# congliuUvA/Clifford-Group-Equivariant-Simplicial-Message-Passing-Networks

Hardware: NVIDIA B200
Metric: simplices/sec fwd+bwd per CSMPN layer (higher is better)
Workload: dtype f32

## Files before the change

clifford-group-equivariant-simplicial-message-passing-networks_b200/csrc/tc_block.cuh:

```cuda
#pragma once
#include "tc_common.cuh"

namespace csmpn {
namespace tcb {
using namespace tc;

constexpr int kTile = 128;
constexpr int kThreads = 512;
constexpr float kInvSqrt2 = 0.70710678118654752440f;

constexpr uint32_t kKH = 2048;
constexpr uint32_t kPS = 2 * kKH + 16;

__host__ __device__ constexpr int round_up(int x, int m) { return (x + m - 1) / m * m; }
__host__ __device__ constexpr int64_t bpt_floats(int B, int64_t rows, int cp) {
  return ((rows + kTile - 1) / kTile) * (int64_t)B * cp * kTile;
}
__device__ __forceinline__ size_t bpt_off(int B, int cp, int64_t tile, int b, int c4, int r) {
  return ((((size_t)tile * B + b) * (cp >> 2) + c4) * kTile + r) * 4;
}

__device__ __forceinline__ float fast_rcp(float x) { float y; asm("rcp.approx.f32 %0, %1;" : "=f"(y) : "f"(x)); return y; }
__device__ __forceinline__ float fast_sqrt(float x) { float y; asm("sqrt.approx.f32 %0, %1;" : "=f"(y) : "f"(x)); return y; }
__device__ __forceinline__ float fast_ex2(float x) { float y; asm("ex2.approx.f32 %0, %1;" : "=f"(y) : "f"(x)); return y; }
__device__ __forceinline__ float fast_sigmoid(float v) { return fast_rcp(1.f + fast_ex2(-1.4426950408889634f * v)); }
__device__ __forceinline__ float fast_sas(float q) { return fast_sqrt(fast_sqrt(fmaf(q, q, kSmoothEps))); }

template <int DIM>
__device__ __forceinline__ void silu_gates(const float* y1, const float* a, const float* b, float* sg, float* inv) {
  using A = Alg<DIM>;
#pragma unroll
  for (int g = 0; g < A::G; ++g) inv[g] = 0.f;
#pragma unroll
  for (int i = 0; i < A::B; ++i) inv[A::grade_of(i)] = fmaf(y1[i], y1[i], inv[A::grade_of(i)]);
  inv[0] = y1[0];
#pragma unroll
  for (int g = 0; g < A::G; ++g) sg[g] = fast_sigmoid(fmaf(a[g], inv[g], b[g]));
}

template <int DIM>
__device__ __forceinline__ void norm_factors(const float* xr, const float* s, float* q, float* nrm, float* rinv) {
  using A = Alg<DIM>;
#pragma unroll
  for (int g = 0; g < A::G; ++g) q[g] = 0.f;
#pragma unroll
  for (int i = 0; i < A::B; ++i) q[A::grade_of(i)] = fmaf(xr[i], xr[i], q[A::grade_of(i)]);
#pragma unroll
  for (int g = 0; g < A::G; ++g) {
    nrm[g] = fast_sas(q[g]);
    rinv[g] = fast_rcp(fmaf(s[g], nrm[g] - 1.f, 1.f) + kEps);
  }
}

template <int DIM>
__device__ __forceinline__ float mv_sumsq(const float* x) {
  float Q = 0.f;
#pragma unroll
  for (int i = 0; i < Alg<DIM>::B; ++i) Q = fmaf(x[i], x[i], Q);
  return Q;
}

struct WJob {
  uint8_t* img0;
  const float* w;
  int c_out, c_in, row0;
};
template <int DIM, bool TRANS, int NJ>
__device__ __forceinline__ void stage_weight_jobs(const WJob (&j)[NJ], int njobs, uint32_t img_bytes, int rows_p, int cols_p,
                                                  uint8_t* zero_base, uint32_t zero_bytes) {
  static_assert(NJ == 1 || NJ == 2, "one or two weights per call");
  constexpr int G = Alg<DIM>::G, U = 4;
  const int lane = threadIdx.x & 31, warp = threadIdx.x >> 5, nwarps = blockDim.x >> 5;
  const int rl = lane >> 2, cl = lane & 3;
  const WJob& j0 = j[0];
  const WJob& j1 = j[NJ - 1];
  const bool two = NJ == 2 && njobs > 1;
  const int R0 = TRANS ? j0.c_in : j0.c_out, C0 = TRANS ? j0.c_out : j0.c_in;
  const int R1 = TRANS ? j1.c_in : j1.c_out, C1 = TRANS ? j1.c_out : j1.c_in;
  const int ncb0 = (C0 + 3) >> 2, ncb1 = (C1 + 3) >> 2;
  const int nb0 = ((R0 + 7) >> 3) * ncb0, nb1 = two ? ((R1 + 7) >> 3) * ncb1 : 0;
  const int total = nb0 + nb1;
  auto decode = [&](int wb, bool& sj, int& row, int& col) -> bool {
    if (wb >= total) return false;
    sj = wb >= nb0;
    if (sj) wb -= nb0;
    const int ncb = sj ? ncb1 : ncb0;
    const int rb = wb / ncb, cb = wb - rb * ncb;
    row = rb * 8 + rl;
    col = cb * 4 + cl;
    return row < (sj ? R1 : R0) && col < (sj ? C1 : C0);
  };
  auto fetch = [&](int wb, float* v) {
#pragma unroll
    for (int g = 0; g < G; ++g) v[g] = 0.f;
    bool sj;
    int row, col;
    if (!decode(wb, sj, row, col)) return;
    const int o = TRANS ? col : row, i = TRANS ? row : col;
    const float* src = (sj ? j1.w : j0.w) + ((size_t)o * (sj ? j1.c_in : j0.c_in) + i) * G;
    if (G == 4 && (reinterpret_cast<uintptr_t>(src) & 15) == 0) {
      const float4 x = __ldg(reinterpret_cast<const float4*>(src));
      v[0] = x.x; v[1] = x.y; v[2] = x.z; v[G - 1] = x.w;
    } else {
#pragma unroll
      for (int g = 0; g < G; ++g) v[g] = __ldg(src + g);
    }
  };
  auto put = [&](int wb, const float* v) {
    bool sj;
    int row, col;
    if (!decode(wb, sj, row, col)) return;
    const int r = (sj ? j1.row0 : j0.row0) + row;
    if (r >= rows_p || col >= cols_p) return;
    uint8_t* dst = (sj ? j1.img0 : j0.img0) + plane_off(rows_p, r, col);
#pragma unroll
    for (int g = 0; g < G; ++g) {
      const float hi = tf32_hi(v[g]);
      *reinterpret_cast<float*>(dst + (size_t)(g * 2 + 0) * img_bytes) = hi;
      *reinterpret_cast<float*>(dst + (size_t)(g * 2 + 1) * img_bytes) = v[g] - hi;
    }
  };
  float x[U][G];
#pragma unroll
  for (int u = 0; u < U; ++u) fetch(warp + u * nwarps, x[u]);
  for (uint32_t i = threadIdx.x; i < (zero_bytes >> 4); i += blockDim.x)
    reinterpret_cast<float4*>(zero_base)[i] = make_float4(0.f, 0.f, 0.f, 0.f);
  __syncthreads();
  for (int base = 0; base < total; base += U * nwarps) {
    float nx[U][G];
    const int nbase = base + U * nwarps;
    if (nbase < total) {
#pragma unroll
      for (int u = 0; u < U; ++u) fetch(nbase + warp + u * nwarps, nx[u]);
    }
#pragma unroll
    for (int u = 0; u < U; ++u) put(base + warp + u * nwarps, x[u]);
    if (nbase < total) {
#pragma unroll
      for (int u = 0; u < U; ++u) {
#pragma unroll
        for (int g = 0; g < G; ++g) x[u][g] = nx[u][g];
      }
    }
  }
}
template <int DIM, bool TRANS>
__device__ __forceinline__ void stage_weight_images(uint8_t* img0, uint32_t img_bytes, const float* __restrict__ w, int c_out,
                                                    int c_in, int rows_p, int cols_p) {
  const WJob j[1] = {{img0, w, c_out, c_in, 0}};
  stage_weight_jobs<DIM, TRANS, 1>(j, 1, img_bytes, rows_p, cols_p, img0, (uint32_t)Alg<DIM>::G * 2u * img_bytes);
}

__device__ __forceinline__ uint64_t chunk_desc(uint32_t half_saddr, int b) {
  return smem_desc(half_saddr + (uint32_t)b * kPS, kKH, 128u);
}

constexpr bool kTf32Truncates = true;
constexpr int kRing = 3;
constexpr int kPipeBars = 3 * kRing + 1;
constexpr int kConvWarps = kThreads / 32 - 1;
constexpr int kConv = kConvWarps * 32;
struct Pipe {
  uint8_t* raw;
  uint8_t* lo;
  uint64_t* load_bar;
  uint64_t* slot_bar;
  uint64_t* full_bar;
  uint64_t* lo_bar;
  uint32_t half;
  __device__ __forceinline__ uint8_t* slot(int q) const { return raw + (size_t)(q % kRing) * half; }
  __device__ __forceinline__ void init(uint8_t* base, uint64_t* bars, uint32_t half_bytes) {
    raw = base; lo = base + (size_t)kRing * half_bytes; half = half_bytes;
    load_bar = bars; slot_bar = bars + kRing; full_bar = bars + 2 * kRing; lo_bar = bars + 3 * kRing;
    if (threadIdx.x == 0) {
      for (int i = 0; i < kPipeBars; ++i) mbar_init(&bars[i], (i >= 2 * kRing && i < 3 * kRing) ? kConvWarps : 1);
      mbar_fence_init();
    }
  }
  __device__ __forceinline__ void conv_done(int q) const {
    fence_async_smem();
    fence_before_sync();
    __syncwarp();
    if ((threadIdx.x & 31) == 0) mbar_arrive(&full_bar[q % kRing]);
  }
  __device__ __forceinline__ void wait_full(int q) const {
    mbar_wait(&full_bar[q % kRing], (q / kRing) & 1);
    fence_after_sync();
  }
};

template <int DIM>
__host__ __device__ constexpr uint32_t wunit_bytes(int rows) { return (uint32_t)Alg<DIM>::G * 2u * (uint32_t)rows * 32u; }

template <int B>
__device__ __forceinline__ void issue_chunk_load_w(const Pipe& p, int q, const float* bpt, int cp, int64_t tile, int kc,
                                                   const uint8_t* wsrc, uint32_t wbytes) {
  const int lane = threadIdx.x & 31;
  uint64_t* bar = &p.load_bar[q % kRing];
  if (lane == 0) mbar_arrive_expect_tx(bar, (bpt ? B * 4096u : 0u) + wbytes);
  __syncwarp();
  if (bpt && lane < B) bulk_g2s(p.slot(q) + lane * kPS, bpt + bpt_off(B, cp, tile, lane, 2 * kc, 0), 4096u, bar);
  if (lane == B) bulk_g2s(p.slot(q) + B * kPS, wsrc, wbytes, bar);
}

struct WPrepArgs {
  const float *w0, *w1;
  int stack, trans, n_real, k_real0, k_real1, np, npass, nk0, nk1;
  float* out;
};
template <int DIM>
__global__ void tc_weight_images_kernel(WPrepArgs a) {
  constexpr int G = Alg<DIM>::G;
  const int R = a.stack ? 2 * a.np : a.np;
  const int nk = a.nk0 + (a.stack ? 0 : a.nk1);
  const int64_t total = (int64_t)a.npass * nk * G * 2 * R * 8;
  for (int64_t e = blockIdx.x * (int64_t)blockDim.x + threadIdx.x; e < total; e += (int64_t)gridDim.x * blockDim.x) {
    const int c = (int)(e & 3), r = (int)((e >> 2) % R), cu = (int)((e / (4 * R)) & 1), hl = (int)((e / (8 * R)) & 1);
    const int g = (int)((e / (16 * R)) % G);
    const int u = (int)(e / ((int64_t)16 * R * G)), ps = u / nk, kc = u % nk;
    const int second_k = (!a.stack && kc >= a.nk0) ? 1 : 0;
    const int k = (second_k ? kc - a.nk0 : kc) * 8 + cu * 4 + c;
    const int k_real = second_k ? a.k_real1 : a.k_real0;
    const float* w = a.stack ? (r < a.np ? a.w0 : a.w1) : (second_k ? a.w1 : a.w0);
    const int n = ps * a.np + (a.stack ? r % a.np : r);
    float x = 0.f;
    if (w && n < a.n_real && k < k_real) x = a.trans ? w[((size_t)k * a.n_real + n) * G + g] : w[((size_t)n * k_real + k) * G + g];
    const float hi = tf32_hi(x);
    a.out[e] = hl ? x - hi : hi;
  }
}
template <int DIM>
__host__ inline int64_t weight_image_floats(int stack, int np, int npass, int nk_total) {
  return (int64_t)npass * nk_total * Alg<DIM>::G * 2 * (stack ? 2 * np : np) * 8;
}

template <int B>
__device__ __forceinline__ void issue_chunk_load(const Pipe& p, int q, const float* bpt, int cp, int64_t tile, int kc) {
  const int lane = threadIdx.x & 31;
  uint64_t* bar = &p.load_bar[q % kRing];
  if (lane == 0) mbar_arrive_expect_tx(bar, B * 4096u);
  __syncwarp();
  if (lane < B) bulk_g2s(p.slot(q) + lane * kPS, bpt + bpt_off(B, cp, tile, lane, 2 * kc, 0), 4096u, bar);
}
template <int B>
__device__ __forceinline__ void split_chunk(const Pipe& p, int q) {
  uint8_t* hi = p.slot(q);
  constexpr int TOT = B * 2 * kTile;
  constexpr int N = (TOT + kConv - 1) / kConv;
  const int ct = (int)threadIdx.x - 32;
  float4 l[N];
#pragma unroll
  for (int i = 0; i < N; ++i) {
    const int it = ct + i * kConv;
    if (it < TOT) {
      const int r = it & (kTile - 1), kh = (it >> 7) & 1, b = it >> 8;
      const uint32_t off = b * kPS + kh * kKH + r * 16;
      const float4 x = *reinterpret_cast<const float4*>(hi + off);
      float4 h;
      split4(x, h, l[i]);
      if (!kTf32Truncates) *reinterpret_cast<float4*>(hi + off) = h;
    }
  }
  if (q >= 1) mbar_wait(p.lo_bar, (q - 1) & 1);
#pragma unroll
  for (int i = 0; i < N; ++i) {
    const int it = ct + i * kConv;
    if (it < TOT) {
      const int r = it & (kTile - 1), kh = (it >> 7) & 1, b = it >> 8;
      *reinterpret_cast<float4*>(p.lo + b * kPS + kh * kKH + r * 16) = l[i];
    }
  }
  p.conv_done(q);
}
template <int DIM>
__device__ __forceinline__ void issue_chunk_mma(const Pipe& p, int q, uint32_t tbase, uint32_t ncols, bool accumulate,
                                                const uint8_t* wimg0, uint32_t img_bytes, int s0, int nsets, uint32_t set_bytes,
                                                uint32_t w_rows, int ks, int n0, uint32_t idesc) {
  using A = Alg<DIM>;
  constexpr int B = A::B;
  const uint64_t a_hi = chunk_desc(smem_addr(p.slot(q)), 0), a_lo = chunk_desc(smem_addr(p.lo), 0);
  const uint64_t w0 = smem_desc(smem_addr(wimg0) + (uint32_t)s0 * set_bytes + 2u * ks * w_rows * 16u + (uint32_t)n0 * 16u,
                                w_rows * 16u, 128u);
  const uint64_t img16 = img_bytes >> 4, set16 = set_bytes >> 4;
  constexpr uint64_t ps16 = kPS >> 4;
#pragma unroll
  for (int s = 0; s < 2; ++s) {
    if (s < nsets) {
#pragma unroll
      for (int b = 0; b < B; ++b)
        mma_tf32_w(tbase + (uint32_t)(s * B + b) * ncols, a_lo + b * ps16, w0 + s * set16 + (2 * A::grade_of(b)) * img16, idesc,
                 accumulate);
    }
  }
  mma_commit_w(p.lo_bar);
#pragma unroll
  for (int s = 0; s < 2; ++s) {
    if (s < nsets) {
#pragma unroll
      for (int b = 0; b < B; ++b) {
        const uint64_t wd = w0 + s * set16 + (2 * A::grade_of(b)) * img16;
        const uint32_t d = tbase + (uint32_t)(s * B + b) * ncols;
        mma_tf32_w(d, a_hi + b * ps16, wd, idesc, 1);
        mma_tf32_w(d, a_hi + b * ps16, wd + img16, idesc, 1);
      }
    }
  }
  mma_commit_w(&p.slot_bar[q % kRing]);
}

}
}
```

clifford-group-equivariant-simplicial-message-passing-networks_b200/csrc/tc_block_bwd.cu:

```cuda
#include <utility>
#include <vector>

#include "tc_block.cuh"

namespace csmpn {
namespace tcb {

struct EwArgs {
  int64_t rows;
  int tiles, C, Cp;
  const float* gy;
  int gy_bpt;
  const int32_t* gy_rows;
  int64_t gy_stride;
  const float *o, *xr, *y2, *y1, *dy2;
  const float *la, *wp, *na, *sa, *sb;
  float *d, *dxr, *dy2p, *dy1;
  float* partial;
};

template <int DIM>
__device__ __forceinline__ void load_mv_bpt(float* v, const float* t, int Cp, int64_t tile, int c4, int r, int j) {
  constexpr int B = Alg<DIM>::B;
#pragma unroll
  for (int b = 0; b < B; ++b) v[b] = t[bpt_off(B, Cp, tile, b, c4, r) + j];
}
template <int DIM>
__device__ __forceinline__ void store_mv_bpt(float* t, const float* v, int Cp, int64_t tile, int c4, int r, int j) {
  constexpr int B = Alg<DIM>::B;
#pragma unroll
  for (int b = 0; b < B; ++b) t[bpt_off(B, Cp, tile, b, c4, r) + j] = v[b];
}

__device__ __forceinline__ void cp_async4(float* dst_smem, const float* src) {
  asm volatile("cp.async.ca.shared.global [%0], [%1], 4;" ::"r"(smem_addr(dst_smem)), "l"(src) : "memory");
}
__device__ __forceinline__ void cp_async_commit() { asm volatile("cp.async.commit_group;" ::: "memory"); }
template <int N>
__device__ __forceinline__ void cp_async_wait() { asm volatile("cp.async.wait_group %0;" ::"n"(N) : "memory"); }

__device__ __forceinline__ void cp_async16(float* dst_smem, const float* src) {
  asm volatile("cp.async.cg.shared.global [%0], [%1], 16;" ::"r"(smem_addr(dst_smem)), "l"(src) : "memory");
}
template <int DIM>
__device__ __forceinline__ void prefetch_mv_bpt(float* st, const float* t, int Cp, int64_t tile, int c4, int r0, int lane) {
  constexpr int B = Alg<DIM>::B;
#pragma unroll
  for (int k = lane; k < B * 8; k += 32) {
    const int b = k >> 3, row = k & 7;
    cp_async16(st + (b * 8 + row) * 4, t + bpt_off(B, Cp, tile, b, c4, r0 + row));
  }
}
template <int DIM>
__device__ __forceinline__ void read_stage(float* v, const float* st, int lane) {
#pragma unroll
  for (int b = 0; b < Alg<DIM>::B; ++b) v[b] = st[b * 32 + lane];
}

template <int DIM, int CP, int CPT>
__global__ void __launch_bounds__(CP * 8, CP <= 32 ? 2 : 1) tc_b1_kernel(EwArgs a) {
  using A = Alg<DIM>;
  constexpr int B = A::B, G = A::G, P = A::P, NP = P + G + 2;
  constexpr int NSLAB = CPT / CP;
  static_assert(CPT % CP == 0, "wide blocks are whole slabs");
  extern __shared__ float sm[];
  constexpr int nw = CP >> 2, nt = CP * 8;
  float* part1 = sm;
  float* part2 = part1 + nw * kTile;
  float* inv_mu_s = part2 + nw * kTile;
  float* dmu_s = inv_mu_s + kTile;
  float* stage = dmu_s + kTile;
  const int tid = threadIdx.x, c4l = tid >> 5, lane = tid & 31, j = lane & 3, rr = lane >> 2;
  const int c4 = (NSLAB > 1 ? (int)blockIdx.y * nw : 0) + c4l;
  const int ch = c4 * 4 + j, C = a.C;
  constexpr int Cp = CPT;
  const bool ch_ok = ch < C;
  float la = ch_ok ? a.la[ch] : 0.f, wv[P], sn[G];
#pragma unroll
  for (int q = 0; q < P; ++q) wv[q] = ch_ok ? a.wp[ch * P + q] : 0.f;
#pragma unroll
  for (int g = 0; g < G; ++g) sn[g] = ch_ok ? sigmoidf_(a.na[ch * G + g]) : 0.f;
  float g_w[P], g_na[G], g_la = 0.f, g_bl = 0.f;
#pragma unroll
  for (int q = 0; q < P; ++q) g_w[q] = 0.f;
#pragma unroll
  for (int g = 0; g < G; ++g) g_na[g] = 0.f;

  constexpr int kIt = kTile / 16;
  constexpr int kIt1 = NSLAB * kIt;
  float* stage_w = stage + (size_t)c4l * (2 * 4 * B * 32);
  auto stage_of = [&](int s, int tensor) { return stage_w + (size_t)(s * 4 + tensor) * B * 32; };
  auto prefetch = [&](int64_t unit, int it, int s) {
    const int64_t tile = unit >> 1;
    const int r0 = (int)(unit & 1) * (kTile / 2) + (it & (kIt - 1)) * 8, r = r0 + rr;
    const int c4x = it < kIt1 ? (it / kIt) * nw + c4l : c4;
    const int chx = c4x * 4 + j;
    __syncwarp();
    prefetch_mv_bpt<DIM>(stage_of(s, 0), a.o, Cp, tile, c4x, r0, lane);
    if (a.gy_bpt) {
      prefetch_mv_bpt<DIM>(stage_of(s, 1), a.gy, Cp, tile, c4x, r0, lane);
    } else {
      float* dst = stage_of(s, 1) + lane;
      if (chx < C && tile * kTile + r < a.rows) {
        const int64_t grow = a.gy_rows ? (int64_t)__ldg(a.gy_rows + tile * kTile + r) : tile * kTile + r;
        const float* src = a.gy + (size_t)grow * a.gy_stride + (size_t)chx * B;
#pragma unroll
        for (int b = 0; b < B; ++b) cp_async4(dst + b * 32, src + b);
      } else {
#pragma unroll
        for (int b = 0; b < B; ++b) dst[b * 32] = 0.f;
      }
    }
    if (it >= kIt1) {
      prefetch_mv_bpt<DIM>(stage_of(s, 2), a.y2, Cp, tile, c4, r0, lane);
      prefetch_mv_bpt<DIM>(stage_of(s, 3), a.xr, Cp, tile, c4, r0, lane);
    }
    cp_async_commit();
  };

  const int64_t n_units = 2 * (int64_t)a.tiles;
  int seq = 0;
  if ((int64_t)blockIdx.x < n_units) prefetch(blockIdx.x, 0, 0);
  for (int64_t unit = blockIdx.x; unit < n_units; unit += gridDim.x) {
    const int64_t tile = unit >> 1;
    const int rbase = (int)(unit & 1) * (kTile / 2);
    const int64_t row0 = tile * kTile;
#pragma unroll 1
    for (int it = 0; it < kIt1 + kIt; ++it, ++seq) {
      if (it + 1 < kIt1 + kIt) prefetch(unit, it + 1, (seq + 1) & 1);
      else if (unit + gridDim.x < n_units) prefetch(unit + gridDim.x, 0, (seq + 1) & 1);
      else cp_async_commit();
      cp_async_wait<1>();
      __syncwarp();
      const int s = seq & 1;
      const int r = rbase + (it & (kIt - 1)) * 8 + rr;
      const bool ok = ch_ok && row0 + r < a.rows;
      if (it < kIt1) {
        const int chx = ((it / kIt) * nw + c4l) * 4 + j;
        const bool okx = chx < C && row0 + r < a.rows;
        const float lax = NSLAB > 1 ? (chx < C ? a.la[chx] : 0.f) : la;
        float o[B], dy[B];
        read_stage<DIM>(o, stage_of(s, 0), lane);
        read_stage<DIM>(dy, stage_of(s, 1), lane);
        float dot = 0.f;
#pragma unroll
        for (int b = 0; b < B; ++b) dot = fmaf(dy[b], o[b], dot);
        float nu = okx ? fast_sas(mv_sumsq<DIM>(o)) : 0.f;
        float dt = okx ? lax * dot : 0.f;
        nu += __shfl_xor_sync(0xffffffffu, nu, 1); dt += __shfl_xor_sync(0xffffffffu, dt, 1);
        nu += __shfl_xor_sync(0xffffffffu, nu, 2); dt += __shfl_xor_sync(0xffffffffu, dt, 2);
        if (j == 0) {
          if (NSLAB > 1 && it >= kIt) { part1[c4l * kTile + r] += nu; part2[c4l * kTile + r] += dt; }
          else { part1[c4l * kTile + r] = nu; part2[c4l * kTile + r] = dt; }
        }
        if (it == kIt1 - 1) {
          __syncthreads();
          if (tid < kTile / 2) {
            const int r2 = rbase + tid;
            float s1 = 0.f, s2 = 0.f;
            for (int w = 0; w < nw; ++w) { s1 += part1[w * kTile + r2]; s2 += part2[w * kTile + r2]; }
            const float inv_mu = 1.f / (s1 / (float)C + kEps);
            inv_mu_s[r2] = inv_mu;
            dmu_s[r2] = -s2 * inv_mu * inv_mu / (float)C;
          }
          __syncthreads();
        }
        continue;
      }
      float dd[B];
      {
        float o[B];
        read_stage<DIM>(o, stage_of(s, 0), lane);
        read_stage<DIM>(dd, stage_of(s, 1), lane);
        const float inv_mu = inv_mu_s[r];
        float dot = 0.f;
#pragma unroll
        for (int b = 0; b < B; ++b) dot = fmaf(dd[b], o[b], dot);
        if (ok) g_la = fmaf(dot, inv_mu, g_la);
        const float Q = mv_sumsq<DIM>(o);
        const float nu = fast_sas(Q);
        const float k1 = la * inv_mu * kInvSqrt2;
        const float k2 = dmu_s[r] * Q * fast_rcp(nu * nu * nu) * kInvSqrt2;
#pragma unroll
        for (int b = 0; b < B; ++b) dd[b] = ok ? fmaf(k1, dd[b], k2 * o[b]) : 0.f;
      }
      store_mv_bpt<DIM>(a.d, dd, Cp, tile, c4, r, j);
      g_bl += dd[0];
      float y2[B], xr[B];
      read_stage<DIM>(y2, stage_of(s, 2), lane);
      read_stage<DIM>(xr, stage_of(s, 3), lane);
      float q[G], nrm[G], rinv[G], xn[B], dxn[B], dy2[B];
      norm_factors<DIM>(xr, sn, q, nrm, rinv);
#pragma unroll
      for (int b = 0; b < B; ++b) { xn[b] = xr[b] * rinv[A::grade_of(b)]; dy2[b] = 0.f; dxn[b] = 0.f; }
      A::template wgp_bwd<false>(y2, xn, wv, dd, nullptr, dy2, dxn, g_w);
      store_mv_bpt<DIM>(a.dy2p, dy2, Cp, tile, c4, r, j);
      float t[G], coef[G];
#pragma unroll
      for (int g = 0; g < G; ++g) t[g] = 0.f;
#pragma unroll
      for (int b = 0; b < B; ++b) t[A::grade_of(b)] = fmaf(dxn[b], xr[b], t[A::grade_of(b)]);
#pragma unroll
      for (int g = 0; g < G; ++g) {
        const float ddn = -t[g] * rinv[g] * rinv[g];
        g_na[g] = fmaf(ddn * (nrm[g] - 1.f), sn[g] * (1.f - sn[g]), g_na[g]);
        coef[g] = ddn * sn[g] * q[g] * fast_rcp(nrm[g] * nrm[g] * nrm[g]);
      }
#pragma unroll
      for (int b = 0; b < B; ++b) dxn[b] = fmaf(dxn[b], rinv[A::grade_of(b)], coef[A::grade_of(b)] * xr[b]);
      store_mv_bpt<DIM>(a.dxr, dxn, Cp, tile, c4, r, j);
    }
  }
  cp_async_wait<0>();
  auto red = [&](float v) {
    v += __shfl_xor_sync(0xffffffffu, v, 4);
    v += __shfl_xor_sync(0xffffffffu, v, 8);
    v += __shfl_xor_sync(0xffffffffu, v, 16);
    return v;
  };
  float* out = a.partial + ((size_t)blockIdx.x * C + (ch_ok ? ch : 0)) * NP;
#pragma unroll
  for (int q = 0; q < P; ++q) { const float v = red(g_w[q]); if (rr == 0 && ch_ok) out[q] = v; }
#pragma unroll
  for (int g = 0; g < G; ++g) { const float v = red(g_na[g]); if (rr == 0 && ch_ok) out[P + g] = v; }
  { const float v = red(g_la); if (rr == 0 && ch_ok) out[P + G] = v; }
  { const float v = red(g_bl); if (rr == 0 && ch_ok) out[P + G + 1] = v; }
}

template <int DIM, int CP, int CPT>
__global__ void __launch_bounds__(CP * 8, CP <= 32 ? 2 : 1) tc_b3_kernel(EwArgs a) {
  using A = Alg<DIM>;
  constexpr int B = A::B, G = A::G, NP = 2 * G + 1;
  extern __shared__ float sm[];
  constexpr int nt = CP * 8;
  float* stage = sm;
  const int tid = threadIdx.x, c4l = tid >> 5, lane = tid & 31, j = lane & 3, rr = lane >> 2;
  const int c4 = (CPT > CP ? (int)blockIdx.y * (CP >> 2) : 0) + c4l;
  const int ch = c4 * 4 + j, C = a.C;
  constexpr int Cp = CPT;
  const bool ch_ok = ch < C;
  float sa[G], sb[G], g_sa[G], g_sb[G], g_b1 = 0.f;
#pragma unroll
  for (int g = 0; g < G; ++g) {
    sa[g] = ch_ok ? a.sa[ch * G + g] : 0.f;
    sb[g] = ch_ok ? a.sb[ch * G + g] : 0.f;
    g_sa[g] = 0.f; g_sb[g] = 0.f;
  }
  constexpr int kIt = kTile / 16;
  float* stage_w = stage + (size_t)c4l * (2 * 2 * B * 32);
  auto stage_of = [&](int s, int tensor) { return stage_w + (size_t)(s * 2 + tensor) * B * 32; };
  auto prefetch = [&](int64_t unit, int it, int s) {
    const int64_t tile = unit >> 1;
    const int r0 = (int)(unit & 1) * (kTile / 2) + it * 8;
    __syncwarp();
    prefetch_mv_bpt<DIM>(stage_of(s, 0), a.y1, Cp, tile, c4, r0, lane);
    prefetch_mv_bpt<DIM>(stage_of(s, 1), a.dy2, Cp, tile, c4, r0, lane);
    cp_async_commit();
  };
  const int64_t n_units = 2 * (int64_t)a.tiles;
  int seq = 0;
  if ((int64_t)blockIdx.x < n_units) prefetch(blockIdx.x, 0, 0);
  for (int64_t unit = blockIdx.x; unit < n_units; unit += gridDim.x) {
    const int64_t tile = unit >> 1;
    const int rbase = (int)(unit & 1) * (kTile / 2);
    const int64_t row0 = tile * kTile;
#pragma unroll 1
    for (int it = 0; it < kIt; ++it, ++seq) {
      if (it + 1 < kIt) prefetch(unit, it + 1, (seq + 1) & 1);
      else if (unit + gridDim.x < n_units) prefetch(unit + gridDim.x, 0, (seq + 1) & 1);
      else cp_async_commit();
      cp_async_wait<1>();
      __syncwarp();
      const int s = seq & 1;
      const int r = rbase + it * 8 + rr;
      const bool ok = ch_ok && row0 + r < a.rows;
      float y1[B], dy[B], sg[G], inv[G], t[G], ds[G];
      read_stage<DIM>(y1, stage_of(s, 0), lane);
      read_stage<DIM>(dy, stage_of(s, 1), lane);
      silu_gates<DIM>(y1, sa, sb, sg, inv);
#pragma unroll
      for (int g = 0; g < G; ++g) t[g] = 0.f;
#pragma unroll
      for (int b = 0; b < B; ++b) t[A::grade_of(b)] = fmaf(dy[b], y1[b], t[A::grade_of(b)]);
#pragma unroll
      for (int g = 0; g < G; ++g) {
        ds[g] = ok ? t[g] * sg[g] * (1.f - sg[g]) : 0.f;
        g_sa[g] = fmaf(ds[g], inv[g], g_sa[g]);
        g_sb[g] += ds[g];
      }
#pragma unroll
      for (int b = 0; b < B; ++b) {
        const int g = A::grade_of(b);
        const float dinv = (g == 0) ? 1.f : 2.f * y1[b];
        dy[b] = ok ? fmaf(sg[g], dy[b], ds[g] * sa[g] * dinv) : 0.f;
      }
      g_b1 += dy[0];
      store_mv_bpt<DIM>(a.dy1, dy, Cp, tile, c4, r, j);
    }
  }
  cp_async_wait<0>();
  auto red = [&](float v) {
    v += __shfl_xor_sync(0xffffffffu, v, 4);
    v += __shfl_xor_sync(0xffffffffu, v, 8);
    v += __shfl_xor_sync(0xffffffffu, v, 16);
    return v;
  };
  float* out = a.partial + ((size_t)blockIdx.x * C + (ch_ok ? ch : 0)) * NP;
#pragma unroll
  for (int g = 0; g < G; ++g) { const float v = red(g_sa[g]); if (rr == 0 && ch_ok) out[g] = v; }
#pragma unroll
  for (int g = 0; g < G; ++g) { const float v = red(g_sb[g]); if (rr == 0 && ch_ok) out[G + g] = v; }
  { const float v = red(g_b1); if (rr == 0 && ch_ok) out[2 * G] = v; }
}

struct GemmArgs {
  int64_t rows;
  int tiles;
  const float* src[2];
  int cp[2], nk[2];
  const float* w[2];
  int wk[2], wn;
  int n16;
  int kmax;
  const float* addend;
  float* out;
  int out_bpt;
  const float *y1, *sa, *sb;
  float* partial;
  int C;
  const float* wimg;
  int np;
};

__device__ __forceinline__ float warp_transpose_reduce16(float (&v)[16], int lane) {
#pragma unroll
  for (int step = 8; step >= 1; step >>= 1) {
    const bool up = (lane & step) != 0;
#pragma unroll
    for (int i = 0; i < step; ++i) {
      const float send = up ? v[i] : v[i + step];
      const float keep = up ? v[i + step] : v[i];
      v[i] = keep + __shfl_xor_sync(0xffffffffu, send, step);
    }
  }
  return v[0] + __shfl_xor_sync(0xffffffffu, v[0], 16);
}
__device__ __forceinline__ float warp_sum(float v) {
#pragma unroll
  for (int o = 16; o >= 1; o >>= 1) v += __shfl_xor_sync(0xffffffffu, v, o);
  return v;
}

template <int DIM, bool SILU, bool ST>
__global__ void __launch_bounds__(kThreads, 1) tc_bgemm_kernel(GemmArgs a) {
  using A = Alg<DIM>;
  constexpr int B = A::B, G = A::G, NPS = 2 * G + 1;
  static_assert(2 * NPS <= 18, "two channels' SiLU gradients are reduced as 16 + 2 values");
  extern __shared__ __align__(1024) uint8_t smem[];
  const int tid = threadIdx.x, warp = uniform_warp_idx(), lane = tid & 31;
  const int nmax = ST ? a.np : (512 / B) / 16 * 16;
  const uint32_t wunit = ST ? wunit_bytes<DIM>(nmax) : 0u;
  const uint32_t half = B * kPS + wunit;
  const uint32_t img = ST ? (uint32_t)nmax * 32u : (uint32_t)a.n16 * a.kmax * 4;
  const uint32_t set_bytes = ST ? 0u : G * 2 * img;
  uint8_t* wimg = smem + (size_t)kRing * half + B * kPS;
  const int nsets = a.src[1] ? 2 : 1;
  uint64_t* bars = reinterpret_cast<uint64_t*>(wimg + (size_t)nsets * set_bytes);
  uint32_t* tmem_slot = reinterpret_cast<uint32_t*>(bars + kPipeBars);
  float* sa_s = reinterpret_cast<float*>(tmem_slot + 4);
  float* sb_s = sa_s + a.n16 * G;
  Pipe p;
  p.init(smem, bars, half);
  if (SILU) {
    for (int i = tid; i < a.n16 * G; i += kThreads) {
      sa_s[i] = (i < a.C * G) ? a.sa[i] : 0.f;
      sb_s[i] = (i < a.C * G) ? a.sb[i] : 0.f;
    }
  }
  float acc[4][2];
#pragma unroll
  for (int it = 0; it < 4; ++it) {
#pragma unroll
    for (int pr = 0; pr < 2; ++pr) acc[it][pr] = 0.f;
  }
  const int npass = (a.n16 + nmax - 1) / nmax;
  const int nk = a.nk[0] + a.nk[1];
  const int per_tile = npass * nk;
  const int my_tiles = (a.tiles - (int)blockIdx.x + (int)gridDim.x - 1) / (int)gridDim.x;
  const int total_chunks = my_tiles * per_tile;
  auto issue = [&](int qq) {
    const int64_t tile = (int64_t)blockIdx.x + (int64_t)(qq / per_tile) * gridDim.x;
    const int kc = (qq % per_tile) % nk;
    const int s = kc < a.nk[0] ? 0 : 1;
    if constexpr (ST) {
      const uint8_t* wsrc = reinterpret_cast<const uint8_t*>(a.wimg) + (size_t)(qq % per_tile) * wunit;
      issue_chunk_load_w<B>(p, qq, a.src[s], a.cp[s], tile, s ? kc - a.nk[0] : kc, wsrc, wunit);
    } else {
      issue_chunk_load<B>(p, qq, a.src[s], a.cp[s], tile, s ? kc - a.nk[0] : kc);
    }
  };
  int q = 0, loaded = 0;
  if (warp == 0) for (; loaded < kRing - 1 && loaded < total_chunks; ++loaded) issue(loaded);
  const uint32_t need = (uint32_t)B * (a.n16 < nmax ? a.n16 : nmax);
  const uint32_t tcols = need <= 32 ? 32 : need <= 64 ? 64 : need <= 128 ? 128 : need <= 256 ? 256 : 512;
  if (warp == 0) tmem_alloc(tmem_slot, tcols);
  if (!ST) {
    {
    const WJob wj[2] = {{wimg, a.w[0], a.wk[0], a.wn, 0}, {wimg + set_bytes, a.w[nsets - 1], a.wk[nsets - 1], a.wn, 0}};
    stage_weight_jobs<DIM, true, 2>(wj, nsets, img, a.n16, a.kmax, wimg, (uint32_t)nsets * set_bytes);
  }
  }
  fence_async_smem();
  fence_before_sync();
  __syncthreads();
  fence_after_sync();
  const uint32_t tbase = *tmem_slot;
  const uint32_t lane_base = (warp & 3) * 32;
  const bool wide_ok = aligned32(a.out);
  for (int t = 0; t < my_tiles; ++t) {
    const int64_t tile = (int64_t)blockIdx.x + (int64_t)t * gridDim.x;
    const int64_t row0 = tile * kTile;
    for (int ps = 0; ps < npass; ++ps) {
      const int n0 = ps * nmax;
      const int Np = (a.n16 - n0) < nmax ? (a.n16 - n0) : nmax;
      const uint32_t idesc = idesc_tf32(kTile, Np, false, false);
      for (int kc = 0; kc < nk; ++kc, ++q) {
        if (warp == 0) {
          p.wait_full(q);
          if (loaded == q + kRing - 1 && loaded < total_chunks) {
            if (q >= 1) mbar_wait(&p.slot_bar[(q - 1) % kRing], ((q - 1) / kRing) & 1);
            issue(loaded);
            ++loaded;
          }
          if constexpr (ST) {
            mbar_wait(&p.load_bar[q % kRing], (q / kRing) & 1);
            issue_chunk_mma<DIM>(p, q, tbase, Np, kc > 0, p.slot(q) + B * kPS, img, 0, 1, 0, nmax, 0, 0, idesc);
          } else {
            const int s = kc < a.nk[0] ? 0 : 1;
            issue_chunk_mma<DIM>(p, q, tbase, Np, kc > 0, wimg, img, s, 1, set_bytes, a.n16, s ? kc - a.nk[0] : kc, n0, idesc);
          }
        } else {
          mbar_wait(&p.load_bar[q % kRing], (q / kRing) & 1);
          split_chunk<B>(p, q);
        }
      }
      const int r = lane_base + lane;
      const bool row_ok = row0 + r < a.rows;
      float4 ad[B];
      if (a.addend && (warp >> 2) < (Np >> 2)) {
#pragma unroll
        for (int b = 0; b < B; ++b) ad[b] = *reinterpret_cast<const float4*>(a.addend + bpt_off(B, a.n16, tile, b, (n0 >> 2) + (warp >> 2), r));
      }
      mbar_wait(&p.slot_bar[(q - 1) % kRing], ((q - 1) / kRing) & 1);
      fence_after_sync();
      if (warp == 0) for (; loaded < q + kRing && loaded < total_chunks; ++loaded) issue(loaded);
      for (int c4 = warp >> 2; c4 < (Np >> 2); c4 += 4) {
        float v[B][4];
#pragma unroll
        for (int b = 0; b < B; ++b) tmem_ld4(tmem_at(tbase, lane_base, b * Np + c4 * 4), v[b]);
        tmem_wait_ld();
        const int gc4 = (n0 >> 2) + c4;
        if (a.addend) {
#pragma unroll
          for (int b = 0; b < B; ++b) {
            v[b][0] += ad[b].x; v[b][1] += ad[b].y; v[b][2] += ad[b].z; v[b][3] += ad[b].w;
          }
          if (c4 + 4 < (Np >> 2)) {
#pragma unroll
            for (int b = 0; b < B; ++b) ad[b] = *reinterpret_cast<const float4*>(a.addend + bpt_off(B, a.n16, tile, b, gc4 + 4, r));
          }
        }
        if constexpr (SILU) {
          const int it = c4 >> 2;
#pragma unroll
          for (int pr = 0; pr < 2; ++pr) {
            float2 y1v[B];
#pragma unroll
            for (int b = 0; b < B; ++b)
              y1v[b] = *reinterpret_cast<const float2*>(a.y1 + bpt_off(B, a.n16, tile, b, gc4, r) + 2 * pr);
            float vals[16], t0 = 0.f, t1 = 0.f;
#pragma unroll
            for (int i = 0; i < 16; ++i) vals[i] = 0.f;
#pragma unroll
            for (int jj = 0; jj < 2; ++jj) {
              const int j = 2 * pr + jj, ch = gc4 * 4 + j;
              float y1[B], dy[B], sg[G], inv[G], tg[G], ds[G];
#pragma unroll
              for (int b = 0; b < B; ++b) {
                y1[b] = jj == 0 ? y1v[b].x : y1v[b].y;
                dy[b] = v[b][j];
              }
              const float* sa = sa_s + ch * G;
              silu_gates<DIM>(y1, sa, sb_s + ch * G, sg, inv);
#pragma unroll
              for (int g = 0; g < G; ++g) tg[g] = 0.f;
#pragma unroll
              for (int b = 0; b < B; ++b) tg[A::grade_of(b)] = fmaf(dy[b], y1[b], tg[A::grade_of(b)]);
              const bool ok = row_ok && ch < a.C;
              float gv[NPS];
#pragma unroll
              for (int g = 0; g < G; ++g) {
                ds[g] = ok ? tg[g] * sg[g] * (1.f - sg[g]) : 0.f;
                gv[g] = ds[g] * inv[g];
                gv[G + g] = ds[g];
              }
#pragma unroll
              for (int b = 0; b < B; ++b) {
                const int g = A::grade_of(b);
                const float dinv = (g == 0) ? 1.f : 2.f * y1[b];
                v[b][j] = ok ? fmaf(sg[g], dy[b], ds[g] * sa[g] * dinv) : 0.f;
              }
              gv[2 * G] = v[0][j];
#pragma unroll
              for (int k = 0; k < NPS; ++k) {
                const int idx = jj * NPS + k;
                if (idx < 16) vals[idx] = gv[k];
                else if (idx == 16) t0 = gv[k];
                else t1 = gv[k];
              }
            }
            const float s16 = warp_transpose_reduce16(vals, lane);
            t0 = warp_sum(t0);
            t1 = warp_sum(t1);
            const float mine = lane < 16 ? s16 : lane == 16 ? t0 : lane == 17 ? t1 : 0.f;
#pragma unroll
            for (int q4 = 0; q4 < 4; ++q4) {
              if (q4 == it) acc[q4][pr] += mine;
            }
          }
        }
        if (a.out_bpt) {
#pragma unroll
          for (int b = 0; b < B; ++b) {
            float4 x = make_float4(v[b][0], v[b][1], v[b][2], v[b][3]);
            if (!row_ok) x = make_float4(0.f, 0.f, 0.f, 0.f);
            *reinterpret_cast<float4*>(a.out + bpt_off(B, a.n16, tile, b, gc4, r)) = x;
          }
        } else if (row_ok) {
#pragma unroll
          for (int jj = 0; jj < 4; ++jj) {
            const int n = gc4 * 4 + jj;
            if (n >= a.wn) continue;
            float* dst = a.out + ((size_t)(row0 + r) * a.wn + n) * B;
            if constexpr (B == 8) {
              if (wide_ok) {
                float w8[8];
#pragma unroll
                for (int b = 0; b < 8; ++b) w8[b] = v[b][jj];
                st_global_v8(dst, w8);
                continue;
              }
            }
#pragma unroll
            for (int h = 0; h < B / 4; ++h)
              *reinterpret_cast<float4*>(dst + 4 * h) = make_float4(v[4 * h][jj], v[4 * h + 1][jj], v[4 * h + 2][jj], v[4 * h + 3][jj]);
          }
        }
      }
      fence_before_sync();
    }
  }
  fence_before_sync();
  __syncthreads();
  if (warp == 0) tmem_dealloc(tbase, tcols);
  if constexpr (SILU) {
    float* red = reinterpret_cast<float*>(p.lo);
#pragma unroll
    for (int it = 0; it < 4; ++it) {
#pragma unroll
      for (int pr = 0; pr < 2; ++pr) {
        float* dst = red + ((warp * 4 + it) * 2 + pr) * 18;
        if (lane < 18) dst[lane] = acc[it][pr];
      }
    }
    __syncthreads();
    for (int e = tid; e < a.C * NPS; e += kThreads) {
      const int ch = e / NPS, k = e - ch * NPS;
      const int c4 = ch >> 2, j = ch & 3, cg = c4 & 3, it = c4 >> 2, pr = j >> 1, idx = (j & 1) * NPS + k;
      float sum = 0.f;
#pragma unroll
      for (int q4 = 0; q4 < 4; ++q4) sum += red[(((cg * 4 + q4) * 4 + it) * 2 + pr) * 18 + idx];
      a.partial[((size_t)blockIdx.x * a.C + ch) * NPS + k] = sum;
    }
  }
}

template <int DIM, bool SILU>
__global__ void __launch_bounds__(kThreads, 1) tc_bgemmdb_kernel(GemmArgs a) {
  using A = Alg<DIM>;
  constexpr int B = A::B, G = A::G, NPS = 2 * G + 1;
  constexpr int kUnits = 6;
  extern __shared__ __align__(1024) uint8_t smem[];
  const int tid = threadIdx.x, warp = uniform_warp_idx(), lane = tid & 31;
  const uint32_t img = (uint32_t)a.n16 * a.kmax * 4;
  const uint32_t set_bytes = G * 2 * img;
  uint8_t* wimg = smem + (kRing + 1) * B * kPS;
  const int nsets = a.src[1] ? 2 : 1;
  uint64_t* bars = reinterpret_cast<uint64_t*>(wimg + (size_t)nsets * set_bytes);
  uint32_t* tmem_slot = reinterpret_cast<uint32_t*>(bars + kPipeBars);
  float* sa_s = reinterpret_cast<float*>(tmem_slot + 4);
  float* sb_s = sa_s + a.n16 * G;
  Pipe p;
  p.init(smem, bars, B * kPS);
  if (SILU) {
    for (int i = tid; i < a.n16 * G; i += kThreads) {
      sa_s[i] = (i < a.C * G) ? a.sa[i] : 0.f;
      sb_s[i] = (i < a.C * G) ? a.sb[i] : 0.f;
    }
  }
  float acc[kUnits][2];
#pragma unroll
  for (int u = 0; u < kUnits; ++u) { acc[u][0] = 0.f; acc[u][1] = 0.f; }
  const int nk = a.nk[0] + a.nk[1];
  const int my_tiles = (a.tiles - (int)blockIdx.x + (int)gridDim.x - 1) / (int)gridDim.x;
  const int total_chunks = my_tiles * nk;
  auto issue = [&](int qq) {
    const int64_t tile = (int64_t)blockIdx.x + (int64_t)(qq / nk) * gridDim.x;
    const int kc = qq % nk;
    const int s = kc < a.nk[0] ? 0 : 1;
    issue_chunk_load<B>(p, qq, a.src[s], a.cp[s], tile, s ? kc - a.nk[0] : kc);
  };
  int q = 0, loaded = 0;
  if (warp == 0) for (; loaded < kRing - 1 && loaded < total_chunks; ++loaded) issue(loaded);
  const int Np = a.n16;
  const uint32_t bufcols = (uint32_t)B * Np;
  const uint32_t need = 2 * bufcols;
  const uint32_t tcols = need <= 32 ? 32 : need <= 64 ? 64 : need <= 128 ? 128 : need <= 256 ? 256 : 512;
  if (warp == 0) tmem_alloc(tmem_slot, tcols);
  {
    const WJob wj[2] = {{wimg, a.w[0], a.wk[0], a.wn, 0}, {wimg + set_bytes, a.w[nsets - 1], a.wk[nsets - 1], a.wn, 0}};
    stage_weight_jobs<DIM, true, 2>(wj, nsets, img, a.n16, a.kmax, wimg, (uint32_t)nsets * set_bytes);
  }
  fence_async_smem();
  fence_before_sync();
  __syncthreads();
  fence_after_sync();
  const uint32_t tbase = *tmem_slot;
  const uint32_t idesc = idesc_tf32(kTile, Np, false, false);
  const uint32_t lane_base = (warp & 3) * 32;
  const int r = lane_base + lane;
  const bool wide_ok = aligned32(a.out);
  const int n_c4 = Np >> 2;

  auto epilogue_unit = [&](int64_t tile, int c4, uint32_t tb) {
    const int64_t row0 = tile * kTile;
    const bool row_ok = row0 + r < a.rows;
    float v[B][4];
#pragma unroll
    for (int b = 0; b < B; ++b) tmem_ld4(tmem_at(tb, lane_base, b * Np + c4 * 4), v[b]);
    if (a.addend) {
      float4 ad[B];
#pragma unroll
      for (int b = 0; b < B; ++b) ad[b] = *reinterpret_cast<const float4*>(a.addend + bpt_off(B, a.n16, tile, b, c4, r));
      tmem_wait_ld();
#pragma unroll
      for (int b = 0; b < B; ++b) {
        v[b][0] += ad[b].x; v[b][1] += ad[b].y; v[b][2] += ad[b].z; v[b][3] += ad[b].w;
      }
    } else {
      tmem_wait_ld();
    }
    if constexpr (SILU) {
      const int u = c4 / 3;
#pragma unroll
      for (int pr = 0; pr < 2; ++pr) {
        float2 y1v[B];
#pragma unroll
        for (int b = 0; b < B; ++b)
          y1v[b] = *reinterpret_cast<const float2*>(a.y1 + bpt_off(B, a.n16, tile, b, c4, r) + 2 * pr);
        float vals[16], t0 = 0.f, t1 = 0.f;
#pragma unroll
        for (int i = 0; i < 16; ++i) vals[i] = 0.f;
#pragma unroll
        for (int jj = 0; jj < 2; ++jj) {
          const int j = 2 * pr + jj, ch = c4 * 4 + j;
          float y1[B], dy[B], sg[G], inv[G], tg[G], ds[G];
#pragma unroll
          for (int b = 0; b < B; ++b) {
            y1[b] = jj == 0 ? y1v[b].x : y1v[b].y;
            dy[b] = v[b][j];
          }
          const float* sa = sa_s + ch * G;
          silu_gates<DIM>(y1, sa, sb_s + ch * G, sg, inv);
#pragma unroll
          for (int g = 0; g < G; ++g) tg[g] = 0.f;
#pragma unroll
          for (int b = 0; b < B; ++b) tg[A::grade_of(b)] = fmaf(dy[b], y1[b], tg[A::grade_of(b)]);
          const bool ok = row_ok && ch < a.C;
          float gv[NPS];
#pragma unroll
          for (int g = 0; g < G; ++g) {
            ds[g] = ok ? tg[g] * sg[g] * (1.f - sg[g]) : 0.f;
            gv[g] = ds[g] * inv[g];
            gv[G + g] = ds[g];
          }
#pragma unroll
          for (int b = 0; b < B; ++b) {
            const int g = A::grade_of(b);
            const float dinv = (g == 0) ? 1.f : 2.f * y1[b];
            v[b][j] = ok ? fmaf(sg[g], dy[b], ds[g] * sa[g] * dinv) : 0.f;
          }
          gv[2 * G] = v[0][j];
#pragma unroll
          for (int k = 0; k < NPS; ++k) {
            const int idx = jj * NPS + k;
            if (idx < 16) vals[idx] = gv[k];
            else if (idx == 16) t0 = gv[k];
            else t1 = gv[k];
          }
        }
        const float s16 = warp_transpose_reduce16(vals, lane);
        t0 = warp_sum(t0);
        t1 = warp_sum(t1);
        const float mine = lane < 16 ? s16 : lane == 16 ? t0 : lane == 17 ? t1 : 0.f;
#pragma unroll
        for (int k = 0; k < kUnits; ++k) {
          if (k == u) acc[k][pr] += mine;
        }
      }
    }
    if (a.out_bpt) {
#pragma unroll
      for (int b = 0; b < B; ++b) {
        float4 x = make_float4(v[b][0], v[b][1], v[b][2], v[b][3]);
        if (!row_ok) x = make_float4(0.f, 0.f, 0.f, 0.f);
        *reinterpret_cast<float4*>(a.out + bpt_off(B, a.n16, tile, b, c4, r)) = x;
      }
    } else if (row_ok) {
#pragma unroll
      for (int jj = 0; jj < 4; ++jj) {
        const int n = c4 * 4 + jj;
        if (n >= a.wn) continue;
        float* dst = a.out + ((size_t)(row0 + r) * a.wn + n) * B;
        if constexpr (B == 8) {
          if (wide_ok) {
            float w8[8];
#pragma unroll
            for (int b = 0; b < 8; ++b) w8[b] = v[b][jj];
            st_global_v8(dst, w8);
            continue;
          }
        }
#pragma unroll
        for (int h = 0; h < B / 4; ++h)
          *reinterpret_cast<float4*>(dst + 4 * h) = make_float4(v[4 * h][jj], v[4 * h + 1][jj], v[4 * h + 2][jj], v[4 * h + 3][jj]);
      }
    }
  };
  int64_t pend_tile = -1;
  int pend_c4 = 0, pend_q = 0;
  uint32_t pend_tb = 0;
  bool pend_ready = false;
  auto epilogue_step = [&]() {
    if (warp < 4 || pend_tile < 0) return;
    if (!pend_ready) {
      mbar_wait(&p.slot_bar[pend_q % kRing], (pend_q / kRing) & 1);
      fence_after_sync();
      pend_ready = true;
    }
    if (pend_c4 < n_c4) {
      epilogue_unit(pend_tile, pend_c4, pend_tb);
      pend_c4 += 3;
    }
    if (pend_c4 >= n_c4) { pend_tile = -1; fence_before_sync(); }
  };

  for (int t = 0; t < my_tiles; ++t) {
    const int64_t tile = (int64_t)blockIdx.x + (int64_t)t * gridDim.x;
    const uint32_t tb = tbase + (uint32_t)(t & 1) * bufcols;
    for (int kc = 0; kc < nk; ++kc, ++q) {
      if (warp == 0) {
        p.wait_full(q);
        if (loaded == q + kRing - 1 && loaded < total_chunks) {
          if (q >= 1) mbar_wait(&p.slot_bar[(q - 1) % kRing], ((q - 1) / kRing) & 1);
          issue(loaded);
          ++loaded;
        }
        const int s = kc < a.nk[0] ? 0 : 1;
        issue_chunk_mma<DIM>(p, q, tb, Np, kc > 0, wimg, img, s, 1, set_bytes, a.n16, s ? kc - a.nk[0] : kc, 0, idesc);
      } else {
        mbar_wait(&p.load_bar[q % kRing], (q / kRing) & 1);
        split_chunk<B>(p, q);
        epilogue_step();
      }
    }
    while (warp >= 4 && pend_tile >= 0) epilogue_step();
    pend_tile = tile; pend_c4 = (warp >> 2) - 1; pend_q = q - 1; pend_tb = tb; pend_ready = false;
  }
  while (warp >= 4 && pend_tile >= 0) epilogue_step();
  fence_before_sync();
  __syncthreads();
  if (warp == 0) tmem_dealloc(tbase, tcols);
  if constexpr (SILU) {
    float* red = reinterpret_cast<float*>(p.lo);
#pragma unroll
    for (int u = 0; u < kUnits; ++u) {
#pragma unroll
      for (int pr = 0; pr < 2; ++pr) {
        float* dst = red + ((warp * kUnits + u) * 2 + pr) * 18;
        if (lane < 18) dst[lane] = acc[u][pr];
      }
    }
    __syncthreads();
    for (int e = tid; e < a.C * NPS; e += kThreads) {
      const int ch = e / NPS, k = e - ch * NPS;
      const int c4 = ch >> 2, j = ch & 3, g3 = c4 % 3, u = c4 / 3, pr = j >> 1, idx = (j & 1) * NPS + k;
      float sum = 0.f;
#pragma unroll
      for (int q4 = 0; q4 < 4; ++q4) sum += red[((((g3 + 1) * 4 + q4) * kUnits + u) * 2 + pr) * 18 + idx];
      a.partial[((size_t)blockIdx.x * a.C + ch) * NPS + k] = sum;
    }
  }
}

struct DwArgs {
  int64_t rows;
  int tiles;
  const float *a0, *a1, *bsrc;
  int cpa, cpb;
  int cpa_total;
  int a_c4;
  int cpb_total;
  int b_c4;
  int M;
  float* partial;
  long long* dbg;
};
long long*& debug_buffer();
#ifdef CSMPN_DEBUG_TOOLS
#define DW_STAMP(code)                                                                       \
  do {                                                                                       \
    if (TL && a.dbg && blockIdx.x == 0 && (tid == 0 || tid == 32) && dbg_n < 250) {          \
      a.dbg[(tid ? 512 : 0) + 2 * dbg_n] = (code);                                           \
      a.dbg[(tid ? 512 : 0) + 2 * dbg_n + 1] = clock64();                                    \
      ++dbg_n;                                                                               \
    }                                                                                        \
  } while (0)
#else
#define DW_STAMP(code) do { } while (0)
#endif

constexpr int kDwRows = 64;
constexpr int kDwLand = 2;
constexpr uint32_t kLand = kTile * 16;

template <int DIM, bool TL>
__global__ void __launch_bounds__(256, 1) tc_dw_kernel(DwArgs a) {
  using A = Alg<DIM>;
  constexpr int B = A::B, G = A::G;
  extern __shared__ __align__(1024) uint8_t smem[];
  const int tid = threadIdx.x, warp = uniform_warp_idx(), lane = tid & 31;
  [[maybe_unused]] int dbg_n = 0;
  const int ca4 = a.cpa >> 2;
  const int na4 = (a.a1 ? 2 : 1) * ca4;
  const int nb4 = a.cpb >> 2;
  const int n4 = na4 + nb4;
  const int ga = a.M / 32, gb = (a.cpb + 31) / 32;
  const uint32_t grp = kDwRows * 128;
  const uint32_t op_bytes = 2u * (ga + gb) * grp;
  uint8_t* ops = smem;
  uint8_t* land = ops + 2 * (size_t)op_bytes;
  const uint32_t land_bytes = (uint32_t)n4 * kLand;
  uint64_t* bars = reinterpret_cast<uint64_t*>(land + (size_t)kDwLand * land_bytes);
  uint64_t* load_bar = bars;
  uint64_t* op_bar = bars + kDwLand;
  uint64_t* full_bar = bars + kDwLand + 2;
  uint32_t* tmem_slot = reinterpret_cast<uint32_t*>(bars + kDwLand + 4);
  constexpr int kConvWarps = 7;
  for (uint32_t i = tid; i < (2 * op_bytes) >> 4; i += 256) reinterpret_cast<float4*>(smem)[i] = make_float4(0.f, 0.f, 0.f, 0.f);
  if (tid == 0) {
    for (int i = 0; i < kDwLand + 2; ++i) mbar_init(&bars[i], 1);
    mbar_init(&full_bar[0], kConvWarps);
    mbar_init(&full_bar[1], kConvWarps);
    mbar_fence_init();
  }
  const bool merged = a.M == 64;
  const uint32_t ncol = merged ? 2u * gb * 32u : (uint32_t)a.cpb;
  const uint32_t need = (uint32_t)G * ncol;
  const uint32_t tcols = need <= 32 ? 32 : need <= 64 ? 64 : need <= 128 ? 128 : need <= 256 ? 256 : 512;
  if (warp == 0) tmem_alloc(tmem_slot, tcols);
  fence_async_smem();
  fence_before_sync();
  __syncthreads();
  fence_after_sync();
  const uint32_t tbase = *tmem_slot;
  const uint32_t idesc = merged ? idesc_tf32(128, (int)ncol, true, true) : idesc_tf32(a.M, a.cpb, true, true);
  const int my_tiles = (a.tiles - (int)blockIdx.x + (int)gridDim.x - 1) / (int)gridDim.x;
  const int steps = my_tiles * B * 2;
  if (warp == 0) {
    const int units = steps >> 1;
    auto issue = [&](int lu) {
      const int64_t tile = (int64_t)blockIdx.x + (int64_t)(lu / B) * gridDim.x;
      const int b = lu % B;
      uint8_t* dst = land + (size_t)(lu % kDwLand) * land_bytes;
      uint64_t* bar = &load_bar[lu % kDwLand];
      if (lane == 0) {
        mbar_arrive_expect_tx(bar, (uint32_t)n4 * kLand);
        bulk_g2s(dst, a.a0 + bpt_off(B, a.cpa_total, tile, b, a.a_c4, 0), (uint32_t)ca4 * kLand, bar);
        if (a.a1) bulk_g2s(dst + (size_t)ca4 * kLand, a.a1 + bpt_off(B, a.cpa_total, tile, b, a.a_c4, 0), (uint32_t)ca4 * kLand, bar);
        bulk_g2s(dst + (size_t)na4 * kLand, a.bsrc + bpt_off(B, a.cpb_total, tile, b, a.b_c4, 0), (uint32_t)nb4 * kLand, bar);
      }
      __syncwarp();
    };
    int loaded = 0;
    for (; loaded < kDwLand && loaded < units; ++loaded) issue(loaded);
    uint32_t grade_used = 0;
    for (int st = 0; st < steps; ++st) {
      const int b = (st >> 1) % B, g = A::grade_of(b);
      DW_STAMP(30);
      mbar_wait(&full_bar[st & 1], (st >> 1) & 1);
      fence_after_sync();
      DW_STAMP(31);
      const uint8_t* op_a = ops + (size_t)(st & 1) * op_bytes;
      const uint8_t* op_b = op_a + 2 * (size_t)ga * grp;
      const uint64_t a_hi = desc_mn32b(smem_addr(op_a), grp, 0), a_lo = a_hi + ((uint64_t)ga * grp >> 4);
      const uint64_t b_hi = desc_mn32b(smem_addr(op_b), grp, 0), b_lo = b_hi + ((uint64_t)gb * grp >> 4);
      const uint32_t dcol = tbase + (uint32_t)g * ncol;
      const uint32_t acc = (grade_used >> g) & 1;
      if (merged) {
#pragma unroll
        for (int ks = 0; ks < kDwRows / 8; ++ks) mma_tf32_w(dcol, a_hi + ks * 64, b_hi + ks * 64, idesc, ks == 0 ? acc : 1u);
      } else {
#pragma unroll
        for (int ks = 0; ks < kDwRows / 8; ++ks) {
          mma_tf32_w(dcol, a_hi + ks * 64, b_hi + ks * 64, idesc, ks == 0 ? acc : 1u);
          mma_tf32_w(dcol, a_hi + ks * 64, b_lo + ks * 64, idesc, 1);
          mma_tf32_w(dcol, a_lo + ks * 64, b_hi + ks * 64, idesc, 1);
        }
      }
      mma_commit_w(&op_bar[st & 1]);
      __syncwarp();
      DW_STAMP(32);
      if ((st & 1) && loaded < units) { issue(loaded); ++loaded; }
      DW_STAMP(33);
      grade_used |= 1u << g;
    }
  } else {
    const int ct = tid - 32, nconv = kConvWarps * 32;
    for (int st = 0; st < steps; ++st) {
      const int lu = st >> 1, rh = st & 1;
      DW_STAMP(40);
      mbar_wait(&load_bar[lu % kDwLand], (lu / kDwLand) & 1);
      DW_STAMP(41);
      if (st >= 2) mbar_wait(&op_bar[st & 1], ((st - 2) >> 1) & 1);
      DW_STAMP(42);
      const uint8_t* src = land + (size_t)(lu % kDwLand) * land_bytes + (uint32_t)rh * (kDwRows * 16);
      uint8_t* op_a = ops + (size_t)(st & 1) * op_bytes;
      uint8_t* op_b = op_a + 2 * (size_t)ga * grp;
      for (int it = ct; it < kDwRows * n4; it += nconv) {
        const int pr = it >> 7, w = it & 127, q = w & 7, g8 = w >> 3;
        const int swap = g8 >> 3, r = ((g8 & 7) << 3) + q;
        const int u = 2 * pr + ((q >> 2) ^ swap);
        const float4 x = *reinterpret_cast<const float4*>(src + (uint32_t)u * kLand + r * 16);
        float4 h, l;
        split4(x, h, l);
        const bool isb = u >= na4;
        const int cc = (isb ? u - na4 : u) * 4;
        uint8_t* base = isb ? op_b : op_a;
        const int ng = isb ? gb : ga;
        const uint32_t off = (uint32_t)(cc >> 5) * grp + mn32b_off(r, cc & 31);
        *reinterpret_cast<float4*>(base + off) = h;
        *reinterpret_cast<float4*>(base + (size_t)ng * grp + off) = l;
      }
      fence_async_smem();
      __syncwarp();
      if (lane == 0) mbar_arrive(&full_bar[st & 1]);
      DW_STAMP(43);
    }
  }
  uint32_t grade_used = 0;
  for (int st = 0; st < steps; ++st) grade_used |= 1u << A::grade_of((st >> 1) % B);
  if (steps > 0) mbar_wait(&op_bar[(steps - 1) & 1], ((steps - 1) >> 1) & 1);
  fence_after_sync();
  if (warp < 4 && merged) {
    const int R = warp * 32 + lane, m = R & 63;
    float* out = a.partial + ((size_t)blockIdx.x * 2 + (R >> 6)) * G * 64 * a.cpb;
    for (int g = 0; g < G; ++g) {
      const bool used = steps > 0 && ((grade_used >> g) & 1);
      for (int n = 0; n < a.cpb; n += 4) {
        float v[4] = {0.f, 0.f, 0.f, 0.f}, w[4] = {0.f, 0.f, 0.f, 0.f};
        if (used) {
          tmem_ld4(tmem_at(tbase, warp * 32, g * ncol + n), v);
          tmem_ld4(tmem_at(tbase, warp * 32, g * ncol + gb * 32 + n), w);
          tmem_wait_ld();
        }
        *reinterpret_cast<float4*>(out + ((size_t)g * 64 + m) * a.cpb + n) = make_float4(v[0] + w[0], v[1] + w[1], v[2] + w[2], v[3] + w[3]);
      }
    }
  } else if (warp < 4) {
    float* out = a.partial + (size_t)blockIdx.x * G * a.M * a.cpb;
    const int m = warp * 32 + lane;
    for (int g = 0; g < G; ++g) {
      const bool used = steps > 0 && ((grade_used >> g) & 1);
      for (int n = 0; n < a.cpb; n += 4) {
        float v[4] = {0.f, 0.f, 0.f, 0.f};
        if (used) {
          tmem_ld4(tmem_at(tbase, warp * 32, g * a.cpb + n), v);
          tmem_wait_ld();
        }
        *reinterpret_cast<float4*>(out + ((size_t)g * a.M + m) * a.cpb + n) = make_float4(v[0], v[1], v[2], v[3]);
      }
    }
  }
  fence_before_sync();
  __syncthreads();
  if (warp == 0) tmem_dealloc(tbase, tcols);
}

struct FinalJob {
  const float* in;
  float* out;
  int parts;
  int64_t stride;
  int kind;
  int n;
  int G, M, N, m0, co, ci;
  int ci_tot, i0, o0;
};
constexpr int kFinalJobs = 14;
struct FinalJobs { FinalJob j[kFinalJobs]; int count; };

__global__ void __launch_bounds__(256) tc_final_kernel(FinalJobs jobs) {
  __shared__ float red[16][17];
  const int e = threadIdx.x & 15, pg = threadIdx.x >> 4;
  int64_t idx = (int64_t)blockIdx.x * 16 + e;
  float s = 0.f;
  float* outp = nullptr;
  for (int k = 0; k < jobs.count; ++k) {
    const FinalJob& jb = jobs.j[k];
    if (idx < jb.n) {
      if (jb.out) {
        size_t src, dst;
        if (jb.kind == 0) {
          src = dst = (size_t)idx;
        } else {
          const int i = (int)(idx % jb.ci), o = (int)((idx / jb.ci) % jb.co), g = (int)(idx / ((int64_t)jb.ci * jb.co));
          src = ((size_t)g * jb.M + jb.m0 + o) * jb.N + i;
          dst = ((size_t)(jb.o0 + o) * jb.ci_tot + jb.i0 + i) * jb.G + g;
        }
        const float* in = jb.in + src;
#pragma unroll 4
        for (int p = pg; p < jb.parts; p += 16) s += in[(size_t)p * jb.stride];
        outp = jb.out + dst;
      }
      break;
    }
    idx -= jb.n;
  }
  red[pg][e] = s;
  __syncthreads();
  if (pg == 0 && outp) {
    float t = 0.f;
#pragma unroll
    for (int i = 0; i < 16; ++i) t += red[i][e];
    *outp = t;
  }
}

template <int DIM>
size_t gemm_smem(int nsets, int n16, int kmax, bool silu = false) {
  constexpr int B = Alg<DIM>::B, G = Alg<DIM>::G;
  return (size_t)(kRing + 1) * B * kPS + (size_t)nsets * G * 2 * n16 * kmax * 4 + 128 + (silu ? (size_t)2 * n16 * G * 4 : 0);
}
inline bool fuse_silu_adjoint() {
  const char* e = getenv("CSMPN_TC_FUSE_SILU");
  return e && e[0] == '1';
}
template <int DIM>
size_t dw_smem(int M, int na4, int cpb) {
  const int ga = M / 32, gb = (cpb + 31) / 32;
  return (size_t)2 * 2 * (ga + gb) * kDwRows * 128 + (size_t)kDwLand * (na4 + cpb / 4) * kLand + 128;
}
constexpr size_t kSmemMax = 227 * 1024;

struct BwdPlan {
  int Cp, cin, n16, tiles;
  int grid_ew, grid_dw;
  int M1, M2;
  int nbw;
  int dw_split;
  int wide, np, n_dwa, n_dwb;
  int64_t img_dy2, img_gx;
  size_t dw_part;
  size_t o_d, o_dxr, o_dy2p, o_dy2, o_dy1, o_p1, o_p3, o_dwa, o_dwb, o_img, total;
};
constexpr int kSlabA = 64, kSlabB = 32;
template <int DIM>
size_t gemm_smem_streamed(int np) {
  constexpr int B = Alg<DIM>::B;
  return (size_t)kRing * (B * kPS + wunit_bytes<DIM>(np)) + (size_t)B * kPS + 128;
}

template <int DIM>
int make_bwd_plan(const csmpn_block_desc& d, BwdPlan* p) {
  constexpr int B = Alg<DIM>::B, G = Alg<DIM>::G, P = Alg<DIM>::P;
  p->Cp = round_up(d.c, 16);
  p->cin = d.c0 + d.c1 + d.c2;
  p->n16 = round_up(p->cin, 16);
  p->tiles = (int)((d.rows + kTile - 1) / kTile);
  p->wide = 0; p->np = 0; p->n_dwa = p->n_dwb = 0; p->img_dy2 = p->img_gx = 0; p->dw_part = 0;
  const int sms = sm_count_cached();
  p->grid_ew = 2 * p->tiles < 2 * sms ? (p->tiles > 0 ? 2 * p->tiles : 1) : 2 * sms;
  p->grid_dw = p->tiles < sms ? (p->tiles > 0 ? p->tiles : 1) : sms;
  bool resident = 2 * B * p->Cp <= 512 && p->Cp <= 64;
  if (resident) {
    p->M1 = 2 * p->Cp <= 64 ? 64 : 128;
    p->M2 = 64;
    p->dw_split = 0;
    if (dw_smem<DIM>(p->M1, 2 * p->Cp / 4, p->Cp) > kSmemMax) { p->dw_split = 1; p->M1 = 64; }
    if (gemm_smem<DIM>(2, p->Cp, p->Cp) > kSmemMax || gemm_smem<DIM>(1, p->n16, p->Cp) > kSmemMax) resident = false;
  }
  if (resident) {
    p->nbw = dw_smem<DIM>(p->M2, p->Cp / 4, p->n16 < 64 ? p->n16 : 64) <= kSmemMax ? 64 : 32;
    const int nb = p->n16 < p->nbw ? p->n16 : p->nbw;
    if (dw_smem<DIM>(p->M1, (p->dw_split ? 1 : 2) * p->Cp / 4, p->Cp) > kSmemMax || dw_smem<DIM>(p->M2, p->Cp / 4, nb) > kSmemMax ||
        p->n16 > 4 * p->nbw)
      resident = false;
  }
  if (!resident) {
    if (!(p->Cp <= 64 || p->Cp == 128 || p->Cp == 256)) return CSMPN_ERR_UNSUPPORTED;
    p->wide = 1;
    p->np = (512 / B) / 16 * 16;
    if (gemm_smem_streamed<DIM>(p->np) > kSmemMax || dw_smem<DIM>(kSlabA, kSlabA / 4, kSlabB) > kSmemMax) return CSMPN_ERR_UNSUPPORTED;
    const int sa = (p->Cp + kSlabA - 1) / kSlabA;
    p->n_dwa = 2 * sa * ((p->Cp + kSlabB - 1) / kSlabB);
    p->n_dwb = sa * ((p->n16 + kSlabB - 1) / kSlabB);
    p->dw_part = (size_t)p->grid_dw * 2 * G * kSlabA * kSlabB;
    p->img_dy2 = weight_image_floats<DIM>(0, p->np, (p->Cp + p->np - 1) / p->np, 2 * (p->Cp / 8));
    p->img_gx = weight_image_floats<DIM>(0, p->np, (p->n16 + p->np - 1) / p->np, p->Cp / 8);
  }
  const size_t t = (size_t)bpt_floats(B, d.rows, p->Cp);
  size_t o = 0;
  p->o_d = o; o += t;
  p->o_dxr = o; o += t;
  p->o_dy2p = o; o += t;
  p->o_dy2 = o; o += t;
  p->o_dy1 = o; o += t;
  auto al = [](size_t x) { return (x + 31) / 32 * 32; };
  p->o_p1 = o; o = al(o + (size_t)p->grid_ew * d.c * (P + G + 2));
  p->o_p3 = o; o = al(o + (size_t)p->grid_ew * d.c * (2 * G + 1));
  if (p->wide) {
    p->o_dwa = o; o += (size_t)p->n_dwa * p->dw_part;
    p->o_dwb = o; o += (size_t)p->n_dwb * p->dw_part;
    p->o_img = o; o += (size_t)((p->img_dy2 + 31) / 32 * 32 + (p->img_gx + 31) / 32 * 32);
  } else {
    p->o_dwa = o; o += (size_t)p->grid_dw * (p->M1 == 64 ? 2 : 1) * G * p->M1 * p->Cp * (p->dw_split ? 2 : 1);
    p->o_dwb = o; o += (size_t)p->grid_dw * 2 * G * p->M2 * p->n16;
    p->o_img = o;
  }
  p->total = o;
  return CSMPN_OK;
}

template <int DIM>
int launch_bwd(const csmpn_block_desc& d, const csmpn_block_grads& g, void* workspace, int64_t bytes, cudaStream_t stream) {
  constexpr int B = Alg<DIM>::B, G = Alg<DIM>::G, P = Alg<DIM>::P;
  BwdPlan p;
  int st = make_bwd_plan<DIM>(d, &p);
  if (st) return st;
  if (!workspace || bytes < (int64_t)(p.total * 4)) return CSMPN_ERR_WORKSPACE;
  if (!d.save_y1 || !d.save_y2 || !d.save_xr || !d.save_o) return CSMPN_ERR_BAD_ARG;
  const float* x0 = d.in_bpt ? d.p0 : d.save_x0;
  if (!x0) return CSMPN_ERR_BAD_ARG;
  if (p.tiles == 0) {
    const size_t c = d.c, cin = p.cin;
    const std::pair<float*, size_t> outs[] = {{g.g_w1, c * cin * G}, {d.has_b1 ? g.g_b1 : nullptr, c}, {g.g_sa, c * G}, {g.g_sb, c * G},
                                              {g.g_wr, c * c * G}, {g.g_na, c * G}, {g.g_wl, c * c * G}, {g.g_bl, c}, {g.g_wp, c * P}, {g.g_la, c}};
    for (const auto& o : outs)
      if (o.first) CSMPN_CUDA_TRY(cudaMemsetAsync(o.first, 0, o.second * sizeof(float), stream));
    return CSMPN_OK;
  }
  float* ws = (float*)workspace;
  const int C = d.c, Cp = p.Cp;
  EwArgs e;
  memset(&e, 0, sizeof(e));
  e.rows = d.rows; e.tiles = p.tiles; e.C = C; e.Cp = Cp;
  e.gy = g.grad_y; e.gy_bpt = g.gy_bpt;
  e.gy_rows = g.gy_bpt ? nullptr : g.gy_rows;
  e.gy_stride = (!g.gy_bpt && g.gy_row_stride > 0) ? g.gy_row_stride : (int64_t)C * Alg<DIM>::B;
  e.o = d.save_o; e.xr = d.save_xr; e.y2 = d.save_y2; e.y1 = d.save_y1;
  e.la = d.la; e.wp = d.wp; e.na = d.na; e.sa = d.sa; e.sb = d.sb;
  e.d = ws + p.o_d; e.dxr = ws + p.o_dxr; e.dy2p = ws + p.o_dy2p; e.dy2 = ws + p.o_dy2; e.dy1 = ws + p.o_dy1;
  e.partial = ws + p.o_p1;
  const int cps = Cp <= 64 ? Cp : 64;
  const int nslab = Cp / cps;
  const int ew_threads = (cps / 4) * 32;
  const dim3 ew_grid(p.grid_ew, nslab);
  const int mask = d.stage_mask ? d.stage_mask : ~0;
  if (mask & 1) {
    const size_t sm1 = (size_t)(2 * (cps / 4) * kTile + 2 * kTile) * 4 + (size_t)2 * 4 * B * ew_threads * 4;
    auto run = [&](auto kern) -> int {
      CSMPN_CUDA_TRY(cudaFuncSetAttribute(kern, cudaFuncAttributeMaxDynamicSharedMemorySize, (int)sm1));
      kern<<<ew_grid, ew_threads, sm1, stream>>>(e);
      return CSMPN_OK;
    };
    int rc = Cp == 16 ? run(tc_b1_kernel<DIM, 16, 16>) : Cp == 32 ? run(tc_b1_kernel<DIM, 32, 32>)
             : Cp == 48 ? run(tc_b1_kernel<DIM, 48, 48>) : Cp == 64 ? run(tc_b1_kernel<DIM, 64, 64>)
             : Cp == 128 ? run(tc_b1_kernel<DIM, 64, 128>) : run(tc_b1_kernel<DIM, 64, 256>);
    if (rc) return rc;
    CSMPN_LAUNCH_CHECK("tc_b1_kernel");
  }
  const int grid = p.tiles < sm_count_cached() ? p.tiles : sm_count_cached();
  float* img_dy2 = ws + p.o_img;
  float* img_gx = img_dy2 + (p.img_dy2 + 31) / 32 * 32;
  GemmArgs ga;
  memset(&ga, 0, sizeof(ga));
  ga.rows = d.rows; ga.tiles = p.tiles;
  ga.src[0] = ws + p.o_d; ga.src[1] = ws + p.o_dxr; ga.cp[0] = ga.cp[1] = Cp; ga.nk[0] = ga.nk[1] = Cp / 8;
  ga.w[0] = d.wl; ga.w[1] = d.wr; ga.wk[0] = ga.wk[1] = C; ga.wn = C;
  ga.n16 = Cp; ga.kmax = Cp;
  ga.addend = ws + p.o_dy2p; ga.out = ws + p.o_dy2; ga.out_bpt = 1;
  const bool fuse_silu = !p.wide && fuse_silu_adjoint() && Cp <= 64 && gemm_smem<DIM>(2, Cp, Cp, true) <= kSmemMax;
  if (fuse_silu) {
    ga.out = ws + p.o_dy1;
    ga.y1 = d.save_y1; ga.sa = d.sa; ga.sb = d.sb; ga.partial = ws + p.o_p3; ga.C = C;
  }
  CSMPN_CUDA_TRY(cudaFuncSetAttribute(tc_bgemm_kernel<DIM, false, false>, cudaFuncAttributeMaxDynamicSharedMemorySize, (int)kSmemMax));
  CSMPN_CUDA_TRY(cudaFuncSetAttribute(tc_bgemm_kernel<DIM, true, false>, cudaFuncAttributeMaxDynamicSharedMemorySize, (int)kSmemMax));
  CSMPN_CUDA_TRY(cudaFuncSetAttribute(tc_bgemm_kernel<DIM, false, true>, cudaFuncAttributeMaxDynamicSharedMemorySize, (int)kSmemMax));
  CSMPN_CUDA_TRY(cudaFuncSetAttribute(tc_bgemmdb_kernel<DIM, false>, cudaFuncAttributeMaxDynamicSharedMemorySize, (int)kSmemMax));
  CSMPN_CUDA_TRY(cudaFuncSetAttribute(tc_bgemmdb_kernel<DIM, true>, cudaFuncAttributeMaxDynamicSharedMemorySize, (int)kSmemMax));
  auto overlap_ok = [&](int n16) {
    const char* e = getenv("CSMPN_TC_OVERLAP");
    return !(e && e[0] == '0') && 2 * B * n16 <= 512 && n16 <= 64;
  };
  auto prep = [&](const WPrepArgs& w, int64_t floats) -> int {
    int64_t blocks = (floats + 255) / 256;
    if (blocks > 4096) blocks = 4096;
    tc_weight_images_kernel<DIM><<<(unsigned)blocks, 256, 0, stream>>>(w);
    CSMPN_LAUNCH_CHECK("tc_weight_images_kernel");
    return CSMPN_OK;
  };
  if (mask & 2) {
    if (p.wide) {
      WPrepArgs w{d.wl, d.wr, 0, 1, C, C, C, p.np, (Cp + p.np - 1) / p.np, Cp / 8, Cp / 8, img_dy2};
      int rc = prep(w, p.img_dy2);
      if (rc) return rc;
      ga.wimg = img_dy2; ga.np = p.np;
      tc_bgemm_kernel<DIM, false, true><<<grid, kThreads, gemm_smem_streamed<DIM>(p.np), stream>>>(ga);
    } else {
      const size_t sm = gemm_smem<DIM>(2, ga.n16, ga.kmax, fuse_silu);
      if (overlap_ok(ga.n16)) {
        if (fuse_silu) tc_bgemmdb_kernel<DIM, true><<<grid, kThreads, sm, stream>>>(ga);
        else tc_bgemmdb_kernel<DIM, false><<<grid, kThreads, sm, stream>>>(ga);
      } else if (fuse_silu) {
        tc_bgemm_kernel<DIM, true, false><<<grid, kThreads, sm, stream>>>(ga);
      } else {
        tc_bgemm_kernel<DIM, false, false><<<grid, kThreads, sm, stream>>>(ga);
      }
    }
    CSMPN_LAUNCH_CHECK("tc_bgemm_kernel(dy2)");
  }
  e.partial = ws + p.o_p3;
  if ((mask & 4) && !fuse_silu) {
    const size_t sm3 = (size_t)2 * 2 * B * ew_threads * 4;
    auto run = [&](auto kern) -> int {
      CSMPN_CUDA_TRY(cudaFuncSetAttribute(kern, cudaFuncAttributeMaxDynamicSharedMemorySize, (int)sm3));
      kern<<<ew_grid, ew_threads, sm3, stream>>>(e);
      return CSMPN_OK;
    };
    int rc = Cp == 16 ? run(tc_b3_kernel<DIM, 16, 16>) : Cp == 32 ? run(tc_b3_kernel<DIM, 32, 32>)
             : Cp == 48 ? run(tc_b3_kernel<DIM, 48, 48>) : Cp == 64 ? run(tc_b3_kernel<DIM, 64, 64>)
             : Cp == 128 ? run(tc_b3_kernel<DIM, 64, 128>) : run(tc_b3_kernel<DIM, 64, 256>);
    if (rc) return rc;
    CSMPN_LAUNCH_CHECK("tc_b3_kernel");
  }
  if (g.grad_x && (mask & 8)) {
    memset(&ga, 0, sizeof(ga));
    ga.rows = d.rows; ga.tiles = p.tiles;
    ga.src[0] = ws + p.o_dy1; ga.cp[0] = Cp; ga.nk[0] = Cp / 8;
    ga.w[0] = d.w1; ga.wk[0] = C; ga.wn = p.cin;
    ga.n16 = p.n16; ga.kmax = Cp;
    ga.out = g.grad_x; ga.out_bpt = g.gx_bpt;
    if (p.wide) {
      WPrepArgs w{d.w1, nullptr, 0, 1, p.cin, C, 0, p.np, (p.n16 + p.np - 1) / p.np, Cp / 8, 0, img_gx};
      int rc = prep(w, p.img_gx);
      if (rc) return rc;
      ga.wimg = img_gx; ga.np = p.np;
      tc_bgemm_kernel<DIM, false, true><<<grid, kThreads, gemm_smem_streamed<DIM>(p.np), stream>>>(ga);
    } else if (overlap_ok(ga.n16)) {
      tc_bgemmdb_kernel<DIM, false><<<grid, kThreads, gemm_smem<DIM>(1, ga.n16, ga.kmax), stream>>>(ga);
    } else {
      tc_bgemm_kernel<DIM, false, false><<<grid, kThreads, gemm_smem<DIM>(1, ga.n16, ga.kmax), stream>>>(ga);
    }
    CSMPN_LAUNCH_CHECK("tc_bgemm_kernel(grad_x)");
  }
  DwArgs da;
  memset(&da, 0, sizeof(da));
  da.dbg = debug_buffer();
#ifdef CSMPN_DEBUG_TOOLS
  auto dw_kernel = da.dbg ? tc_dw_kernel<DIM, true> : tc_dw_kernel<DIM, false>;
#else
  auto dw_kernel = tc_dw_kernel<DIM, false>;
#endif
  CSMPN_CUDA_TRY(cudaFuncSetAttribute(dw_kernel, cudaFuncAttributeMaxDynamicSharedMemorySize, (int)kSmemMax));
  da.rows = d.rows; da.tiles = p.tiles;
  std::vector<FinalJob> jobs;
  auto wjob = [&](const float* in, float* out, int parts, int M, int N, int m0, int co, int ci, int ci_tot, int i0, int o0) {
    if (co <= 0 || ci <= 0 || !out) return;
    FinalJob jb;
    memset(&jb, 0, sizeof(jb));
    jb.in = in; jb.out = out; jb.parts = parts; jb.stride = (int64_t)G * M * N; jb.kind = 1; jb.n = co * ci * G;
    jb.G = G; jb.M = M; jb.N = N; jb.m0 = m0; jb.co = co; jb.ci = ci; jb.ci_tot = ci_tot; jb.i0 = i0; jb.o0 = o0;
    jobs.push_back(jb);
  };
  auto clampi = [](int v, int hi) { return v < 0 ? 0 : (v > hi ? hi : v); };
  if (p.wide) {
    const size_t smw = dw_smem<DIM>(kSlabA, kSlabA / 4, kSlabB);
    da.M = kSlabA; da.a1 = nullptr;
    int li = 0;
    for (int which = 0; which < 2; ++which) {
      for (int ma = 0; ma < Cp; ma += kSlabA) {
        const int ca = (Cp - ma) < kSlabA ? (Cp - ma) : kSlabA;
        for (int nb = 0; nb < Cp; nb += kSlabB, ++li) {
          float* part = ws + p.o_dwa + (size_t)li * p.dw_part;
          if (mask & 16) {
            da.a0 = ws + (which ? p.o_dxr : p.o_d); da.cpa = ca; da.cpa_total = Cp; da.a_c4 = ma / 4;
            da.bsrc = d.save_y2; da.cpb = kSlabB; da.cpb_total = Cp; da.b_c4 = nb / 4;
            da.partial = part;
            dw_kernel<<<p.grid_dw, 256, smw, stream>>>(da);
            CSMPN_LAUNCH_CHECK("tc_dw_kernel(wl,wr slab)");
          }
          wjob(part, which ? g.g_wr : g.g_wl, p.grid_dw * 2, kSlabA, kSlabB, 0, clampi(C - ma, ca), clampi(C - nb, kSlabB), C, nb, ma);
        }
      }
    }
    li = 0;
    for (int ma = 0; ma < Cp; ma += kSlabA) {
      const int ca = (Cp - ma) < kSlabA ? (Cp - ma) : kSlabA;
      for (int nb = 0; nb < p.n16; nb += kSlabB, ++li) {
        const int cb = (p.n16 - nb) < kSlabB ? (p.n16 - nb) : kSlabB;
        float* part = ws + p.o_dwb + (size_t)li * p.dw_part;
        if (mask & 32) {
          da.a0 = ws + p.o_dy1; da.cpa = ca; da.cpa_total = Cp; da.a_c4 = ma / 4;
          da.bsrc = x0; da.cpb = cb; da.cpb_total = p.n16; da.b_c4 = nb / 4;
          da.partial = part;
          dw_kernel<<<p.grid_dw, 256, dw_smem<DIM>(kSlabA, kSlabA / 4, cb), stream>>>(da);
          CSMPN_LAUNCH_CHECK("tc_dw_kernel(w1 slab)");
        }
        wjob(part, g.g_w1, p.grid_dw * 2, kSlabA, cb, 0, clampi(C - ma, ca), clampi(p.cin - nb, cb), p.cin, nb, ma);
      }
    }
  } else {
    da.a0 = ws + p.o_d; da.a1 = ws + p.o_dxr; da.cpa = Cp; da.cpa_total = Cp; da.a_c4 = 0;
    da.bsrc = d.save_y2; da.cpb = Cp; da.cpb_total = Cp; da.b_c4 = 0;
    da.M = p.M1;
    da.partial = ws + p.o_dwa;
    const int pa = p.M1 == 64 ? 2 : 1;
    const size_t dwa_part = (size_t)p.grid_dw * pa * G * p.M1 * Cp;
    if (!(mask & 16)) {
    } else if (!p.dw_split) {
      dw_kernel<<<p.grid_dw, 256, dw_smem<DIM>(da.M, 2 * Cp / 4, Cp), stream>>>(da);
      CSMPN_LAUNCH_CHECK("tc_dw_kernel(wl,wr)");
    } else {
      da.a1 = nullptr;
      dw_kernel<<<p.grid_dw, 256, dw_smem<DIM>(da.M, Cp / 4, Cp), stream>>>(da);
      CSMPN_LAUNCH_CHECK("tc_dw_kernel(wl)");
      da.a0 = ws + p.o_dxr;
      da.partial = ws + p.o_dwa + dwa_part;
      dw_kernel<<<p.grid_dw, 256, dw_smem<DIM>(da.M, Cp / 4, Cp), stream>>>(da);
      CSMPN_LAUNCH_CHECK("tc_dw_kernel(wr)");
    }
    for (int i0 = 0; i0 < p.n16 && (mask & 32); i0 += p.nbw) {
      const int nb = (p.n16 - i0) < p.nbw ? (p.n16 - i0) : p.nbw;
      da.a0 = ws + p.o_dy1; da.a1 = nullptr; da.cpa = Cp; da.cpa_total = Cp; da.a_c4 = 0;
      da.bsrc = x0; da.cpb = nb; da.cpb_total = p.n16; da.b_c4 = i0 / 4;
      da.M = p.M2;
      da.partial = ws + p.o_dwb + (size_t)p.grid_dw * 2 * G * p.M2 * i0;
      dw_kernel<<<p.grid_dw, 256, dw_smem<DIM>(da.M, Cp / 4, nb), stream>>>(da);
      CSMPN_LAUNCH_CHECK("tc_dw_kernel(w1)");
    }
    wjob(ws + p.o_dwa, g.g_wl, p.grid_dw * pa, p.M1, Cp, 0, C, C, C, 0, 0);
    if (!p.dw_split) wjob(ws + p.o_dwa, g.g_wr, p.grid_dw * pa, p.M1, Cp, Cp, C, C, C, 0, 0);
    else wjob(ws + p.o_dwa + dwa_part, g.g_wr, p.grid_dw * pa, p.M1, Cp, 0, C, C, C, 0, 0);
    for (int i0 = 0; i0 < p.cin; i0 += p.nbw) {
      const int nb = (p.n16 - i0) < p.nbw ? (p.n16 - i0) : p.nbw;
      const int ci = (p.cin - i0) < p.nbw ? (p.cin - i0) : p.nbw;
      wjob(ws + p.o_dwb + (size_t)p.grid_dw * 2 * G * p.M2 * i0, g.g_w1, p.grid_dw * 2, p.M2, nb, 0, C, ci, p.cin, i0, 0);
    }
  }
  auto cjob = [&](const float* in, float* out, int parts, int NPk, int col0, int width) {
    FinalJob jb;
    memset(&jb, 0, sizeof(jb));
    jb.in = in + col0; jb.out = out; jb.parts = parts; jb.stride = (int64_t)C * NPk; jb.kind = 1; jb.n = C * width;
    jb.G = 1; jb.M = C; jb.N = NPk; jb.m0 = 0; jb.co = C; jb.ci = width; jb.ci_tot = width; jb.i0 = 0; jb.o0 = 0;
    jobs.push_back(jb);
  };
  const int NP1 = P + G + 2, NP3 = 2 * G + 1;
  cjob(ws + p.o_p1, g.g_wp, p.grid_ew, NP1, 0, P);
  cjob(ws + p.o_p1, g.g_na, p.grid_ew, NP1, P, G);
  cjob(ws + p.o_p1, g.g_la, p.grid_ew, NP1, P + G, 1);
  cjob(ws + p.o_p1, g.g_bl, p.grid_ew, NP1, P + G + 1, 1);
  const int parts3 = fuse_silu ? grid : p.grid_ew;
  cjob(ws + p.o_p3, g.g_sa, parts3, NP3, 0, G);
  cjob(ws + p.o_p3, g.g_sb, parts3, NP3, G, G);
  cjob(ws + p.o_p3, d.has_b1 ? g.g_b1 : nullptr, parts3, NP3, 2 * G, 1);
  if (mask & 64) {
    for (size_t j0 = 0; j0 < jobs.size(); j0 += kFinalJobs) {
      FinalJobs fj;
      memset(&fj, 0, sizeof(fj));
      int64_t total = 0;
      for (size_t k = j0; k < jobs.size() && k < j0 + kFinalJobs; ++k) {
        fj.j[fj.count++] = jobs[k];
        total += jobs[k].n;
      }
      tc_final_kernel<<<(unsigned)((total + 15) / 16), 256, 0, stream>>>(fj);
      CSMPN_LAUNCH_CHECK("tc_final_kernel");
    }
  }
  return CSMPN_OK;
}

template <int DIM>
int64_t bwd_ws_bytes(const csmpn_block_desc& d) {
  BwdPlan p;
  if (make_bwd_plan<DIM>(d, &p)) return -1;
  return (int64_t)(p.total * 4);
}

}

int tc_block_bwd(int dim, const csmpn_block_desc* d, const csmpn_block_grads* g, void* ws, int64_t bytes, cudaStream_t stream) {
  if (dim == 2) return tcb::launch_bwd<2>(*d, *g, ws, bytes, stream);
  if (dim == 3) return tcb::launch_bwd<3>(*d, *g, ws, bytes, stream);
  return CSMPN_ERR_UNSUPPORTED;
}
bool tc_block_bwd_supported(int dim, int c_in, int c) {
  csmpn_block_desc d;
  memset(&d, 0, sizeof(d));
  d.c0 = c_in; d.c = c; d.rows = 128;
  tcb::BwdPlan p;
  if (dim == 2) return tcb::make_bwd_plan<2>(d, &p) == CSMPN_OK;
  if (dim == 3) return tcb::make_bwd_plan<3>(d, &p) == CSMPN_OK;
  return false;
}
int tc_block_bwd_wide(int dim, int c_in, int c) {
  csmpn_block_desc d;
  memset(&d, 0, sizeof(d));
  d.c0 = c_in; d.c = c; d.rows = 128;
  tcb::BwdPlan p;
  const int st = dim == 2 ? tcb::make_bwd_plan<2>(d, &p) : dim == 3 ? tcb::make_bwd_plan<3>(d, &p) : -1;
  return st == CSMPN_OK && p.wide;
}
int64_t tc_block_bwd_workspace(int dim, const csmpn_block_desc* d) {
  if (dim == 2) return tcb::bwd_ws_bytes<2>(*d);
  if (dim == 3) return tcb::bwd_ws_bytes<3>(*d);
  return -1;
}

}
```

clifford-group-equivariant-simplicial-message-passing-networks_b200/csrc/tc_block_fwd.cu:

```cuda
#include "tc_block.cuh"

namespace csmpn {
namespace tcb {

struct FwdArgs {
  int64_t rows;
  int tiles;
  int C, Cp;
  int cin, kin8;
  int in_bpt, in_cp;
  int mode, c0, c1, c2, pair_attr;
  int vt_k, vt_fp;
  const float *p0, *p1, *p2;
  const int32_t *src, *dst, *eid;
  const float *w1, *b1, *sa, *sb, *wr, *na, *wl, *bl, *wp, *la;
  float *save_y1, *y2, *save_xr, *save_o, *save_x0;
  float* y;
  const float* res;
  int out_bpt, has_b1;
  const float *wimg1, *wimg2;
  int ns1, ns2;
  long long* dbg;
};
#ifdef CSMPN_DEBUG_TOOLS
#define TSTAMP(code)                                                                         \
  do {                                                                                       \
    if (TL && a.dbg && blockIdx.x == 0 && (tid == 0 || tid == 64) && dbg_n < 250) {          \
      a.dbg[(tid ? 512 : 0) + 2 * dbg_n] = (code);                                           \
      a.dbg[(tid ? 512 : 0) + 2 * dbg_n + 1] = clock64();                                    \
      ++dbg_n;                                                                               \
    }                                                                                        \
  } while (0)
#else
#define TSTAMP(code) do { } while (0)
#endif

template <int DIM>
struct ApiItems {
  static constexpr int H = Alg<DIM>::B / 4, PPR = 8 * H, TOT = kTile * PPR, N = (TOT + kConv - 1) / kConv;
  __device__ static __forceinline__ void decode(int it, int& r, int& cl, int& h) {
    const int l = it & 31, g = it >> 5;
    h = l % H;
    const int clo = (l / H) & 3, rlo = l / (4 * H);
    cl = (g & 1) * 4 + clo;
    r = (g >> 1) * (8 / H) + rlo;
  }
};

template <int DIM>
struct GatherIdx {
  int32_t d[ApiItems<DIM>::N], s[ApiItems<DIM>::N], e[ApiItems<DIM>::N];
};
template <int DIM>
__device__ __forceinline__ void load_gather_idx(const FwdArgs& a, int64_t row0, GatherIdx<DIM>& gi) {
  constexpr int N = ApiItems<DIM>::N, TOT = ApiItems<DIM>::TOT;
  if (a.mode == 0) return;
  const int ct = (int)threadIdx.x - 32;
#pragma unroll
  for (int i = 0; i < N; ++i) {
    const int it = ct + i * kConv;
    int r, cl, h;
    ApiItems<DIM>::decode(it, r, cl, h);
    const int64_t R = row0 + r;
    const bool ok = it < TOT && R < a.rows;
    if (a.mode == 2) {
      gi.d[i] = ok ? a.src[R * a.vt_k] : 0;
      gi.s[i] = (ok && a.vt_k > 1) ? a.src[R * a.vt_k + 1] : 0;
      gi.e[i] = (ok && a.vt_k > 2) ? a.src[R * a.vt_k + 2] : 0;
    } else {
      gi.d[i] = ok ? a.dst[R] : 0;
      gi.s[i] = ok ? a.src[R] : 0;
      gi.e[i] = (ok && a.c1 > 0 && !a.pair_attr) ? a.eid[R] : 0;
    }
  }
}

template <int DIM>
__device__ __forceinline__ void gather_chunk_api(const FwdArgs& a, int64_t row0, int kc, float4* v, const GatherIdx<DIM>& gi) {
  constexpr int B = Alg<DIM>::B, H = ApiItems<DIM>::H, PPR = ApiItems<DIM>::PPR, N = ApiItems<DIM>::N, TOT = ApiItems<DIM>::TOT;
  const int ct = (int)threadIdx.x - 32;
#pragma unroll
  for (int i = 0; i < N; ++i) {
    const int it = ct + i * kConv;
    int r, cl, h;
    ApiItems<DIM>::decode(it, r, cl, h);
    const int c = kc * 8 + cl;
    const int64_t R = row0 + r;
    v[i] = make_float4(0.f, 0.f, 0.f, 0.f);
    if (it < TOT && R < a.rows && c < a.cin) {
      if (a.mode == 2) {
        const int kf = a.vt_k * a.vt_fp, t = c / kf, j = (c - t * kf) / a.vt_fp, f = c - t * kf - j * a.vt_fp;
        const int64_t vrow = j == 0 ? gi.d[i] : j == 1 ? gi.s[i] : gi.e[i];
        v[i] = __ldg(reinterpret_cast<const float4*>(a.p0 + (vrow * (a.c0 / a.vt_k) + t * a.vt_fp + f) * B + 4 * h));
      } else if (a.mode == 1) {
        if (c < a.c0) {
          const int64_t d = gi.d[i], s = gi.s[i];
          const float4 x = __ldg(reinterpret_cast<const float4*>(a.p0 + (d * a.c0 + c) * B + 4 * h));
          const float4 z = __ldg(reinterpret_cast<const float4*>(a.p0 + (s * a.c0 + c) * B + 4 * h));
          v[i] = make_float4(x.x - z.x, x.y - z.y, x.z - z.z, x.w - z.w);
        } else if (a.pair_attr) {
          const int k = c - a.c0, half = a.c1 >> 1;
          const int64_t n = k < half ? gi.s[i] : gi.d[i];
          v[i] = __ldg(reinterpret_cast<const float4*>(a.p1 + (n * half + (k < half ? k : k - half)) * B + 4 * h));
        } else {
          const int64_t e = gi.e[i];
          v[i] = __ldg(reinterpret_cast<const float4*>(a.p1 + (e * a.c1 + (c - a.c0)) * B + 4 * h));
        }
      } else {
        if (c < a.c0) v[i] = __ldg(reinterpret_cast<const float4*>(a.p0 + (R * a.c0 + c) * B + 4 * h));
        else if (c < a.c0 + a.c1) v[i] = __ldg(reinterpret_cast<const float4*>(a.p1 + (R * a.c1 + (c - a.c0)) * B + 4 * h));
        else v[i] = __ldg(reinterpret_cast<const float4*>(a.p2 + (R * a.c2 + (c - a.c0 - a.c1)) * B + 4 * h));
      }
    }
  }
}
template <int DIM>
__device__ __forceinline__ void store_chunk_api(const Pipe& p, int q, const float4* v, float* x0, int x0_cp, int64_t tile, int kc) {
  constexpr int B = Alg<DIM>::B;
  constexpr int H = ApiItems<DIM>::H, PPR = ApiItems<DIM>::PPR, N = ApiItems<DIM>::N, TOT = ApiItems<DIM>::TOT;
  const int ct = (int)threadIdx.x - 32;
  uint8_t* hi = p.slot(q);
  uint8_t* lo = p.lo;
  float4 lv[N];
#pragma unroll
  for (int i = 0; i < N; ++i) {
    const int it = ct + i * kConv;
    if (it < TOT) {
      int r, cl, h;
      ApiItems<DIM>::decode(it, r, cl, h);
      float4 hv;
      split4(v[i], hv, lv[i]);
      const uint32_t off = (4 * h) * kPS + (cl >> 2) * kKH + r * 16 + (cl & 3) * 4;
      *reinterpret_cast<float*>(hi + off) = hv.x;
      *reinterpret_cast<float*>(hi + off + kPS) = hv.y;
      *reinterpret_cast<float*>(hi + off + 2 * kPS) = hv.z;
      *reinterpret_cast<float*>(hi + off + 3 * kPS) = hv.w;
    }
  }
  if (x0) {
#pragma unroll
    for (int i = 0; i < N; ++i) {
      const int it = ct + i * kConv;
      if (it < TOT) {
        int r, cl, h;
        ApiItems<DIM>::decode(it, r, cl, h);
        float* dst = x0 + bpt_off(B, x0_cp, tile, 4 * h, 2 * kc + (cl >> 2), r) + (cl & 3);
        const size_t bs = (size_t)(x0_cp >> 2) * kTile * 4;
        dst[0] = v[i].x;
        dst[bs] = v[i].y;
        dst[2 * bs] = v[i].z;
        dst[3 * bs] = v[i].w;
      }
    }
  }
  if (q >= 1) mbar_wait(p.lo_bar, (q - 1) & 1);
#pragma unroll
  for (int i = 0; i < N; ++i) {
    const int it = ct + i * kConv;
    if (it < TOT) {
      int r, cl, h;
      ApiItems<DIM>::decode(it, r, cl, h);
      const uint32_t off = (4 * h) * kPS + (cl >> 2) * kKH + r * 16 + (cl & 3) * 4;
      *reinterpret_cast<float*>(lo + off) = lv[i].x;
      *reinterpret_cast<float*>(lo + off + kPS) = lv[i].y;
      *reinterpret_cast<float*>(lo + off + 2 * kPS) = lv[i].z;
      *reinterpret_cast<float*>(lo + off + 3 * kPS) = lv[i].w;
    }
  }
}
__device__ __forceinline__ void conv_barrier() { asm volatile("bar.sync 1, %0;" ::"n"(kConv) : "memory"); }
template <int B>
__device__ __forceinline__ void zero_chunk_bpt(float* dst, int cp, int64_t tile, int kc) {
  for (int it = (int)threadIdx.x - 32; it < B * 2 * kTile; it += kConv) {
    const int r = it & (kTile - 1), kh = (it >> 7) & 1, b = it >> 8;
    *reinterpret_cast<float4*>(dst + bpt_off(B, cp, tile, b, 2 * kc + kh, r)) = make_float4(0.f, 0.f, 0.f, 0.f);
  }
}

template <int DIM, bool BPT_IN, bool ST>
__global__ void __launch_bounds__(kThreads, 1) tc_f1_kernel(FwdArgs a) {
  using A = Alg<DIM>;
  constexpr int B = A::B, G = A::G;
  constexpr bool LOADS = BPT_IN || ST;
  extern __shared__ __align__(1024) uint8_t smem[];
  const int tid = threadIdx.x, warp = uniform_warp_idx(), lane = tid & 31;
  const int C = a.C, Cp = a.Cp, nk = a.kin8 / 8;
  const int NS = ST ? a.ns1 : Cp;
  const int npass = ST ? Cp / NS : 1;
  const uint32_t wunit = ST ? wunit_bytes<DIM>(NS) : 0u;
  const uint32_t half = B * kPS + wunit;
  const uint32_t img = ST ? (uint32_t)NS * 32u : (uint32_t)a.kin8 * Cp * 4;
  uint8_t* wimg = smem + (size_t)kRing * half + B * kPS;
  float* b1_s = reinterpret_cast<float*>(wimg + (ST ? 0 : (size_t)G * 2 * img));
  float* sa_s = b1_s + Cp;
  float* sb_s = sa_s + Cp * G;
  uint64_t* bars = reinterpret_cast<uint64_t*>(sb_s + Cp * G);
  uint32_t* tmem_slot = reinterpret_cast<uint32_t*>(bars + kPipeBars);
  Pipe p;
  p.init(smem, bars, half);
  const int my_tiles = (a.tiles - (int)blockIdx.x + (int)gridDim.x - 1) / (int)gridDim.x;
  const int per_tile = npass * nk;
  const int total_chunks = my_tiles * per_tile;
  auto tile_of = [&](int q) { return (int64_t)blockIdx.x + (int64_t)(q / per_tile) * gridDim.x; };
  auto load = [&](int qq) {
    if constexpr (ST) {
      const uint8_t* wsrc = reinterpret_cast<const uint8_t*>(a.wimg1) + (size_t)(qq % per_tile) * wunit;
      issue_chunk_load_w<B>(p, qq, BPT_IN ? a.p0 : nullptr, a.in_cp, tile_of(qq), qq % nk, wsrc, wunit);
    } else {
      issue_chunk_load<B>(p, qq, a.p0, a.in_cp, tile_of(qq), qq % nk);
    }
  };
  int q = 0;
  int loaded = 0;
  float4 gv[BPT_IN ? 1 : ApiItems<DIM>::N];
  GatherIdx<DIM> gi;
  if (!BPT_IN && warp != 0 && total_chunks > 0) {
    load_gather_idx<DIM>(a, tile_of(0) * kTile, gi);
    gather_chunk_api<DIM>(a, tile_of(0) * kTile, 0, gv, gi);
  }
  if (LOADS && warp == 0) {
    for (; loaded < kRing - 1 && loaded < total_chunks; ++loaded) load(loaded);
  }

  const uint32_t need = (uint32_t)B * NS;
  const uint32_t tcols = need <= 32 ? 32 : need <= 64 ? 64 : need <= 128 ? 128 : need <= 256 ? 256 : 512;
  if (warp == 0) tmem_alloc(tmem_slot, tcols);
  const float pf_b1 = (tid < C && a.has_b1) ? __ldg(a.b1 + tid) : 0.f;
  const float pf_sa = tid < C * G ? __ldg(a.sa + tid) : 0.f;
  const float pf_sb = tid < C * G ? __ldg(a.sb + tid) : 0.f;
  if (!ST) stage_weight_images<DIM, false>(wimg, img, a.w1, C, a.cin, Cp, a.kin8);
  if (tid < Cp) b1_s[tid] = pf_b1;
  for (int i = tid + kThreads; i < Cp; i += kThreads) b1_s[i] = (i < C && a.has_b1) ? a.b1[i] : 0.f;
  if (tid < Cp * G) { sa_s[tid] = pf_sa; sb_s[tid] = pf_sb; }
  for (int i = tid + kThreads; i < Cp * G; i += kThreads) {
    sa_s[i] = (i < C * G) ? a.sa[i] : 0.f;
    sb_s[i] = (i < C * G) ? a.sb[i] : 0.f;
  }
  fence_async_smem();
  fence_before_sync();
  __syncthreads();
  fence_after_sync();
  const uint32_t tbase = *tmem_slot;
  const uint32_t idesc = idesc_tf32(kTile, NS, false, false);
  for (int t = 0; t < my_tiles; ++t) {
    const int64_t tile = (int64_t)blockIdx.x + (int64_t)t * gridDim.x;
    const int64_t row0 = tile * kTile;
    for (int ps = 0; ps < npass; ++ps) {
      const int n0 = ps * NS;
      for (int kc = 0; kc < nk; ++kc, ++q) {
        if (warp == 0) {
          p.wait_full(q);
          if (LOADS && loaded == q + kRing - 1 && loaded < total_chunks) {
            if (q >= 1) mbar_wait(&p.slot_bar[(q - 1) % kRing], ((q - 1) / kRing) & 1);
            load(loaded);
            ++loaded;
          }
          if constexpr (ST) {
            mbar_wait(&p.load_bar[q % kRing], (q / kRing) & 1);
            issue_chunk_mma<DIM>(p, q, tbase, NS, kc > 0, p.slot(q) + B * kPS, img, 0, 1, 0, NS, 0, 0, idesc);
          } else {
            issue_chunk_mma<DIM>(p, q, tbase, Cp, kc > 0, wimg, img, 0, 1, 0, Cp, kc, 0, idesc);
          }
        } else if (BPT_IN) {
          mbar_wait(&p.load_bar[q % kRing], (q / kRing) & 1);
          split_chunk<B>(p, q);
        } else {
          if (q >= kRing) mbar_wait(&p.slot_bar[q % kRing], ((q - kRing) / kRing) & 1);
          float* x0 = ps == 0 ? a.save_x0 : nullptr;
          store_chunk_api<DIM>(p, q, gv, x0, round_up(a.kin8, 16), tile, kc);
          p.conv_done(q);
          if (q + 1 < total_chunks) {
            if ((q + 1) % per_tile == 0) load_gather_idx<DIM>(a, tile_of(q + 1) * kTile, gi);
            gather_chunk_api<DIM>(a, tile_of(q + 1) * kTile, (q + 1) % nk, gv, gi);
          }
          if (x0 && kc == nk - 1 && (a.kin8 & 8)) zero_chunk_bpt<B>(x0, round_up(a.kin8, 16), tile, nk);
        }
      }
      mbar_wait(&p.slot_bar[(q - 1) % kRing], ((q - 1) / kRing) & 1);
      fence_after_sync();
      if (LOADS && warp == 0) {
        for (; loaded < q + kRing && loaded < total_chunks; ++loaded) load(loaded);
      }
      const int r = (warp & 3) * 32 + lane;
      const bool row_ok = row0 + r < a.rows;
      for (int c4 = warp >> 2; c4 < (NS >> 2); c4 += 4) {
        const int gc4 = (n0 >> 2) + c4;
        float v[B][4];
#pragma unroll
        for (int b = 0; b < B; ++b) tmem_ld4(tmem_at(tbase, (warp & 3) * 32, b * NS + c4 * 4), v[b]);
        tmem_wait_ld();
#pragma unroll
        for (int j = 0; j < 4; ++j) {
          const int ch = gc4 * 4 + j;
          float y1[B];
          const bool ok = row_ok && ch < C;
#pragma unroll
          for (int b = 0; b < B; ++b) y1[b] = ok ? v[b][j] : 0.f;
          if (ok) y1[0] += b1_s[ch];
#pragma unroll
          for (int b = 0; b < B; ++b) v[b][j] = y1[b];
        }
        if (a.save_y1) {
#pragma unroll
          for (int b = 0; b < B; ++b)
            *reinterpret_cast<float4*>(a.save_y1 + bpt_off(B, Cp, tile, b, gc4, r)) = make_float4(v[b][0], v[b][1], v[b][2], v[b][3]);
        }
#pragma unroll
        for (int j = 0; j < 4; ++j) {
          const int ch = gc4 * 4 + j;
          float y1[B], sg[G], inv[G];
#pragma unroll
          for (int b = 0; b < B; ++b) y1[b] = v[b][j];
          silu_gates<DIM>(y1, sa_s + ch * G, sb_s + ch * G, sg, inv);
#pragma unroll
          for (int b = 0; b < B; ++b) v[b][j] = y1[b] * sg[A::grade_of(b)];
        }
#pragma unroll
        for (int b = 0; b < B; ++b)
          *reinterpret_cast<float4*>(a.y2 + bpt_off(B, Cp, tile, b, gc4, r)) = make_float4(v[b][0], v[b][1], v[b][2], v[b][3]);
      }
      fence_before_sync();
    }
  }
  fence_before_sync();
  __syncthreads();
  if (warp == 0) tmem_dealloc(tbase, tcols);
}

template <int DIM, bool BPT_IN>
__global__ void __launch_bounds__(kThreads, 1) tc_f1db_kernel(FwdArgs a) {
  using A = Alg<DIM>;
  [[maybe_unused]] constexpr bool TL = true;
  [[maybe_unused]] int dbg_n = 0;
  constexpr int B = A::B, G = A::G;
  extern __shared__ __align__(1024) uint8_t smem[];
  const int tid = threadIdx.x, warp = uniform_warp_idx(), lane = tid & 31;
  const int C = a.C, Cp = a.Cp, nk = a.kin8 / 8;
  const uint32_t img = (uint32_t)a.kin8 * Cp * 4;
  uint8_t* wimg = smem + (kRing + 1) * B * kPS;
  float* b1_s = reinterpret_cast<float*>(wimg + (size_t)G * 2 * img);
  float* sa_s = b1_s + Cp;
  float* sb_s = sa_s + Cp * G;
  uint64_t* bars = reinterpret_cast<uint64_t*>(sb_s + Cp * G);
  uint32_t* tmem_slot = reinterpret_cast<uint32_t*>(bars + kPipeBars);
  Pipe p;
  p.init(smem, bars, B * kPS);
  const int my_tiles = (a.tiles - (int)blockIdx.x + (int)gridDim.x - 1) / (int)gridDim.x;
  const int total_chunks = my_tiles * nk;
  auto tile_of = [&](int q) { return (int64_t)blockIdx.x + (int64_t)(q / nk) * gridDim.x; };
  int q = 0, loaded = 0;
  float4 gv[BPT_IN ? 1 : ApiItems<DIM>::N];
  GatherIdx<DIM> gi;
  if (!BPT_IN && warp != 0 && total_chunks > 0) {
    load_gather_idx<DIM>(a, tile_of(0) * kTile, gi);
    gather_chunk_api<DIM>(a, tile_of(0) * kTile, 0, gv, gi);
  }
  if (BPT_IN && warp == 0) {
    for (; loaded < kRing - 1 && loaded < total_chunks; ++loaded)
      issue_chunk_load<B>(p, loaded, a.p0, a.in_cp, tile_of(loaded), loaded % nk);
  }

  const uint32_t bufcols = (uint32_t)B * Cp;
  const uint32_t need = 2 * bufcols;
  const uint32_t tcols = need <= 32 ? 32 : need <= 64 ? 64 : need <= 128 ? 128 : need <= 256 ? 256 : 512;
  if (warp == 0) tmem_alloc(tmem_slot, tcols);
  const float pf_b1 = (tid < C && a.has_b1) ? __ldg(a.b1 + tid) : 0.f;
  const float pf_sa = tid < C * G ? __ldg(a.sa + tid) : 0.f;
  const float pf_sb = tid < C * G ? __ldg(a.sb + tid) : 0.f;
  stage_weight_images<DIM, false>(wimg, img, a.w1, C, a.cin, Cp, a.kin8);
  if (tid < Cp) b1_s[tid] = pf_b1;
  for (int i = tid + kThreads; i < Cp; i += kThreads) b1_s[i] = (i < C && a.has_b1) ? a.b1[i] : 0.f;
  if (tid < Cp * G) { sa_s[tid] = pf_sa; sb_s[tid] = pf_sb; }
  for (int i = tid + kThreads; i < Cp * G; i += kThreads) {
    sa_s[i] = (i < C * G) ? a.sa[i] : 0.f;
    sb_s[i] = (i < C * G) ? a.sb[i] : 0.f;
  }
  fence_async_smem();
  fence_before_sync();
  __syncthreads();
  fence_after_sync();
  const uint32_t tbase = *tmem_slot;
  const uint32_t idesc = idesc_tf32(kTile, Cp, false, false);
  const int r = (warp & 3) * 32 + lane;
  const int n_c4 = Cp >> 2;

  auto epilogue_unit = [&](int64_t tile, int c4, uint32_t tb) {
    const bool row_ok = tile * kTile + r < a.rows;
    float v[B][4];
#pragma unroll
    for (int b = 0; b < B; ++b) tmem_ld4(tmem_at(tb, (warp & 3) * 32, b * Cp + c4 * 4), v[b]);
    tmem_wait_ld();
#pragma unroll
    for (int j = 0; j < 4; ++j) {
      const int ch = c4 * 4 + j;
      float y1[B];
      const bool ok = row_ok && ch < C;
#pragma unroll
      for (int b = 0; b < B; ++b) y1[b] = ok ? v[b][j] : 0.f;
      if (ok) y1[0] += b1_s[ch];
#pragma unroll
      for (int b = 0; b < B; ++b) v[b][j] = y1[b];
    }
    if (a.save_y1) {
#pragma unroll
      for (int b = 0; b < B; ++b)
        *reinterpret_cast<float4*>(a.save_y1 + bpt_off(B, Cp, tile, b, c4, r)) = make_float4(v[b][0], v[b][1], v[b][2], v[b][3]);
    }
#pragma unroll
    for (int j = 0; j < 4; ++j) {
      const int ch = c4 * 4 + j;
      float y1[B], sg[G], inv[G];
#pragma unroll
      for (int b = 0; b < B; ++b) y1[b] = v[b][j];
      silu_gates<DIM>(y1, sa_s + ch * G, sb_s + ch * G, sg, inv);
#pragma unroll
      for (int b = 0; b < B; ++b) v[b][j] = y1[b] * sg[A::grade_of(b)];
    }
#pragma unroll
    for (int b = 0; b < B; ++b)
      *reinterpret_cast<float4*>(a.y2 + bpt_off(B, Cp, tile, b, c4, r)) = make_float4(v[b][0], v[b][1], v[b][2], v[b][3]);
  };
  int64_t pend_tile = -1;
  int pend_c4 = 0, pend_q = 0;
  uint32_t pend_tb = 0;
  bool pend_ready = false;
  auto epilogue_step = [&]() {
    if (warp < 4 || pend_tile < 0) return;
    if (!pend_ready) {
      mbar_wait(&p.slot_bar[pend_q % kRing], (pend_q / kRing) & 1);
      fence_after_sync();
      pend_ready = true;
    }
    if (pend_c4 < n_c4) {
      epilogue_unit(pend_tile, pend_c4, pend_tb);
      pend_c4 += 3;
    }
    if (pend_c4 >= n_c4) { pend_tile = -1; fence_before_sync(); }
  };

  for (int t = 0; t < my_tiles; ++t) {
    const int64_t tile = (int64_t)blockIdx.x + (int64_t)t * gridDim.x;
    const uint32_t tb = tbase + (uint32_t)(t & 1) * bufcols;
    for (int kc = 0; kc < nk; ++kc, ++q) {
      if (warp == 0) {
        TSTAMP(36);
        p.wait_full(q);
        TSTAMP(37);
        if (BPT_IN && loaded == q + kRing - 1 && loaded < total_chunks) {
          if (q >= 1) mbar_wait(&p.slot_bar[(q - 1) % kRing], ((q - 1) / kRing) & 1);
          issue_chunk_load<B>(p, loaded, a.p0, a.in_cp, tile_of(loaded), loaded % nk);
          ++loaded;
        }
        issue_chunk_mma<DIM>(p, q, tb, Cp, kc > 0, wimg, img, 0, 1, 0, Cp, kc, 0, idesc);
        TSTAMP(38);
      } else {
        if (BPT_IN) {
          mbar_wait(&p.load_bar[q % kRing], (q / kRing) & 1);
          split_chunk<B>(p, q);
        } else {
          TSTAMP(30);
          if (q >= kRing) mbar_wait(&p.slot_bar[q % kRing], ((q - kRing) / kRing) & 1);
          TSTAMP(31);
          store_chunk_api<DIM>(p, q, gv, a.save_x0, round_up(a.kin8, 16), tile, kc);
          TSTAMP(32);
          p.conv_done(q);
          TSTAMP(33);
          if (q + 1 < total_chunks) {
            if ((q + 1) % nk == 0) load_gather_idx<DIM>(a, tile_of(q + 1) * kTile, gi);
            gather_chunk_api<DIM>(a, tile_of(q + 1) * kTile, (q + 1) % nk, gv, gi);
          }
          if (a.save_x0 && kc == nk - 1 && (a.kin8 & 8)) zero_chunk_bpt<B>(a.save_x0, round_up(a.kin8, 16), tile, nk);
          TSTAMP(34);
        }
        epilogue_step();
        TSTAMP(35);
      }
    }
    while (warp >= 4 && pend_tile >= 0) epilogue_step();
    pend_tile = tile; pend_c4 = (warp >> 2) - 1; pend_q = q - 1; pend_tb = tb; pend_ready = false;
  }
  while (warp >= 4 && pend_tile >= 0) epilogue_step();
  fence_before_sync();
  __syncthreads();
  if (warp == 0) tmem_dealloc(tbase, tcols);
}

template <int DIM, bool TL, bool ST>
__global__ void __launch_bounds__(kThreads, 1) tc_f2_kernel(FwdArgs a) {
  using A = Alg<DIM>;
  constexpr int B = A::B, G = A::G, P = A::P;
  extern __shared__ __align__(1024) uint8_t smem[];
  const int tid = threadIdx.x, warp = uniform_warp_idx(), lane = tid & 31;
  [[maybe_unused]] int dbg_n = 0;
  TSTAMP(2);
  const int C = a.C, Cp = a.Cp, nk = Cp / 8;
  const int NS = ST ? a.ns2 : Cp;
  const int npass = ST ? Cp / NS : 1;
  const uint32_t wunit = ST ? wunit_bytes<DIM>(2 * NS) : 0u;
  const uint32_t half = B * kPS + wunit;
  const uint32_t img = ST ? (uint32_t)2 * NS * 32u : (uint32_t)2 * Cp * Cp * 4;
  const uint32_t set_bytes = ST ? 0u : G * 2 * img;
  uint8_t* wimg = smem + (size_t)kRing * half + B * kPS;
  float* sn_s = reinterpret_cast<float*>(wimg + (size_t)set_bytes);
  float* wv_s = sn_s + Cp * G;
  float* bl_s = wv_s + Cp * P;
  float* la_s = bl_s + Cp;
  float* rowsum_s = la_s + Cp;
  uint64_t* bars = reinterpret_cast<uint64_t*>(rowsum_s + 8 * kTile);
  uint32_t* tmem_slot = reinterpret_cast<uint32_t*>(bars + kPipeBars);
  Pipe p;
  p.init(smem, bars, half);
  const int my_tiles = (a.tiles - (int)blockIdx.x + (int)gridDim.x - 1) / (int)gridDim.x;
  const int per_tile = npass * nk;
  const int total_chunks = my_tiles * per_tile;
  auto tile_of = [&](int q) { return (int64_t)blockIdx.x + (int64_t)(q / per_tile) * gridDim.x; };
  auto load = [&](int qq) {
    if constexpr (ST) {
      const uint8_t* wsrc = reinterpret_cast<const uint8_t*>(a.wimg2) + (size_t)(qq % per_tile) * wunit;
      issue_chunk_load_w<B>(p, qq, a.y2, Cp, tile_of(qq), qq % nk, wsrc, wunit);
    } else {
      issue_chunk_load<B>(p, qq, a.y2, Cp, tile_of(qq), qq % nk);
    }
  };
  int q = 0, loaded = 0;
  if (warp == 0) {
    for (; loaded < kRing - 1 && loaded < total_chunks; ++loaded) load(loaded);
  }

  TSTAMP(3);
  const uint32_t need = 2 * B * NS;
  const uint32_t tcols = need <= 32 ? 32 : need <= 64 ? 64 : need <= 128 ? 128 : need <= 256 ? 256 : 512;
  if (warp == 0) tmem_alloc(tmem_slot, tcols);
  const float pf_na = tid < C * G ? __ldg(a.na + tid) : 0.f;
  const float pf_wp0 = tid < C * P ? __ldg(a.wp + tid) : 0.f;
  const float pf_wp1 = tid + kThreads < C * P ? __ldg(a.wp + tid + kThreads) : 0.f;
  const float pf_bl = tid < C ? __ldg(a.bl + tid) : 0.f;
  const float pf_la = tid < C ? __ldg(a.la + tid) : 0.f;
  if (!ST) {
    const WJob wj[2] = {{wimg, a.wr, C, C, 0}, {wimg, a.wl, C, C, Cp}};
    stage_weight_jobs<DIM, false, 2>(wj, 2, img, 2 * Cp, Cp, wimg, (uint32_t)G * 2u * img);
  }
  TSTAMP(4);
  if (tid < Cp * G) sn_s[tid] = tid < C * G ? sigmoidf_(pf_na) : 0.f;
  for (int i = tid + kThreads; i < Cp * G; i += kThreads) sn_s[i] = (i < C * G) ? sigmoidf_(a.na[i]) : 0.f;
  if (tid < Cp * P) wv_s[tid] = pf_wp0;
  if (tid + kThreads < Cp * P) wv_s[tid + kThreads] = pf_wp1;
  for (int i = tid + 2 * kThreads; i < Cp * P; i += kThreads) wv_s[i] = (i < C * P) ? a.wp[i] : 0.f;
  if (tid < Cp) { bl_s[tid] = pf_bl; la_s[tid] = pf_la; }
  for (int i = tid + kThreads; i < Cp; i += kThreads) {
    bl_s[i] = (i < C) ? a.bl[i] : 0.f;
    la_s[i] = (i < C) ? a.la[i] : 0.f;
  }
  fence_async_smem();
  fence_before_sync();
  __syncthreads();
  fence_after_sync();
  const uint32_t tbase = *tmem_slot;
  const uint32_t idesc = idesc_tf32(kTile, 2 * NS, false, false);
  const uint32_t col_r = 0, col_l = NS, bcols = 2 * NS;
  const bool wide_ok = aligned32(a.y) && (!a.res || aligned32(a.res));
  const uint32_t lane_base = (warp & 3) * 32;

  TSTAMP(1);
  for (int t = 0; t < my_tiles; ++t) {
    const int64_t tile = (int64_t)blockIdx.x + (int64_t)t * gridDim.x;
    const int64_t row0 = tile * kTile;
    const int r = lane_base + lane;
    const bool row_ok = row0 + r < a.rows;
    float rs = 0.f;
    for (int ps = 0; ps < npass; ++ps) {
      const int n0 = ps * NS;
      for (int kc = 0; kc < nk; ++kc, ++q) {
        TSTAMP(10);
        if (warp == 0) {
          p.wait_full(q);
          TSTAMP(14);
          if (loaded == q + kRing - 1 && loaded < total_chunks) {
            if (q >= 1) mbar_wait(&p.slot_bar[(q - 1) % kRing], ((q - 1) / kRing) & 1);
            load(loaded);
            ++loaded;
          }
          TSTAMP(16);
          if constexpr (ST) issue_chunk_mma<DIM>(p, q, tbase, bcols, kc > 0, p.slot(q) + B * kPS, img, 0, 1, 0, bcols, 0, 0, idesc);
          else issue_chunk_mma<DIM>(p, q, tbase, bcols, kc > 0, wimg, img, 0, 1, 0, bcols, kc, 0, idesc);
          TSTAMP(15);
        } else {
          mbar_wait(&p.load_bar[q % kRing], (q / kRing) & 1);
          TSTAMP(11);
          split_chunk<B>(p, q);
          TSTAMP(13);
        }
      }
      TSTAMP(20);
      float4 y2v[B];
      if ((warp >> 2) < (NS >> 2)) {
#pragma unroll
        for (int b = 0; b < B; ++b) y2v[b] = *reinterpret_cast<const float4*>(a.y2 + bpt_off(B, Cp, tile, b, (n0 >> 2) + (warp >> 2), r));
      }
      mbar_wait(&p.slot_bar[(q - 1) % kRing], ((q - 1) / kRing) & 1);
      fence_after_sync();
      TSTAMP(21);
      if (warp == 0) {
        for (; loaded < q + kRing && loaded < total_chunks; ++loaded) load(loaded);
      }
      for (int c4 = warp >> 2; c4 < (NS >> 2); c4 += 4) {
        const int gc4 = (n0 >> 2) + c4;
        float xr[B][4], o[B][4];
        if (c4 != (warp >> 2)) {
#pragma unroll
          for (int b = 0; b < B; ++b) y2v[b] = *reinterpret_cast<const float4*>(a.y2 + bpt_off(B, Cp, tile, b, gc4, r));
        }
#pragma unroll
        for (int b = 0; b < B; ++b) tmem_ld4(tmem_at(tbase, lane_base, b * bcols + col_r + c4 * 4), xr[b]);
#pragma unroll
        for (int b = 0; b < B; ++b) tmem_ld4(tmem_at(tbase, lane_base, b * bcols + col_l + c4 * 4), o[b]);
        tmem_wait_ld();
        if (a.save_xr) {
#pragma unroll
          for (int b = 0; b < B; ++b) {
            float4 x = make_float4(xr[b][0], xr[b][1], xr[b][2], xr[b][3]);
            if (!row_ok) x = make_float4(0.f, 0.f, 0.f, 0.f);
            *reinterpret_cast<float4*>(a.save_xr + bpt_off(B, Cp, tile, b, gc4, r)) = x;
          }
        }
#pragma unroll
        for (int j = 0; j < 4; ++j) {
          const int ch = gc4 * 4 + j;
          float xn[B], oj[B], y2[B], qv[G], nrm[G], rinv[G];
#pragma unroll
          for (int b = 0; b < B; ++b) { xn[b] = xr[b][j]; oj[b] = o[b][j]; }
#pragma unroll
          for (int b = 0; b < B; ++b) y2[b] = j == 0 ? y2v[b].x : j == 1 ? y2v[b].y : j == 2 ? y2v[b].z : y2v[b].w;
          norm_factors<DIM>(xn, sn_s + ch * G, qv, nrm, rinv);
#pragma unroll
          for (int b = 0; b < B; ++b) xn[b] *= rinv[A::grade_of(b)];
          oj[0] += bl_s[ch];
          A::template wgp<false>(y2, xn, wv_s + ch * P, nullptr, oj);
          const bool ok = row_ok && ch < C;
#pragma unroll
          for (int b = 0; b < B; ++b) oj[b] = ok ? oj[b] * kInvSqrt2 : 0.f;
          if (ok) rs += fast_sas(mv_sumsq<DIM>(oj));
#pragma unroll
          for (int b = 0; b < B; ++b) o[b][j] = oj[b];
        }
        if constexpr (!ST) {
#pragma unroll
          for (int b = 0; b < B; ++b) tmem_st4(tmem_at(tbase, lane_base, b * bcols + col_l + c4 * 4), o[b]);
        }
        if (ST || a.save_o) {
#pragma unroll
          for (int b = 0; b < B; ++b)
            *reinterpret_cast<float4*>(a.save_o + bpt_off(B, Cp, tile, b, gc4, r)) = make_float4(o[b][0], o[b][1], o[b][2], o[b][3]);
        }
      }
      if constexpr (!ST) tmem_wait_st();
      fence_before_sync();
    }
    TSTAMP(22);
    float* rowsum_t = rowsum_s + (t & 1) * 4 * kTile;
    rowsum_t[(warp >> 2) * kTile + r] = rs;
    __syncthreads();
    TSTAMP(23);
    const float inv_mu = fast_rcp((rowsum_t[r] + rowsum_t[kTile + r] + rowsum_t[2 * kTile + r] + rowsum_t[3 * kTile + r]) / (float)C + kEps);
    for (int gc4 = warp >> 2; gc4 < (Cp >> 2); gc4 += 4) {
      float o[B][4];
      if constexpr (ST) {
#pragma unroll
        for (int b = 0; b < B; ++b) {
          const float4 x = *reinterpret_cast<const float4*>(a.save_o + bpt_off(B, Cp, tile, b, gc4, r));
          o[b][0] = x.x; o[b][1] = x.y; o[b][2] = x.z; o[b][3] = x.w;
        }
      } else {
#pragma unroll
        for (int b = 0; b < B; ++b) tmem_ld4(tmem_at(tbase, lane_base, b * bcols + col_l + gc4 * 4), o[b]);
        tmem_wait_ld();
      }
#pragma unroll
      for (int j = 0; j < 4; ++j) {
        const float sc = la_s[gc4 * 4 + j] * inv_mu;
#pragma unroll
        for (int b = 0; b < B; ++b) o[b][j] *= sc;
      }
      if (a.out_bpt) {
#pragma unroll
        for (int b = 0; b < B; ++b)
          *reinterpret_cast<float4*>(a.y + bpt_off(B, Cp, tile, b, gc4, r)) = make_float4(o[b][0], o[b][1], o[b][2], o[b][3]);
      } else if (row_ok) {
#pragma unroll
        for (int j = 0; j < 4; ++j) {
          const int ch = gc4 * 4 + j;
          if (ch >= C) continue;
          const size_t off = ((size_t)(row0 + r) * C + ch) * B;
          if constexpr (B == 8) {
            if (wide_ok) {
              float v[8];
#pragma unroll
              for (int b = 0; b < 8; ++b) v[b] = o[b][j];
              if (a.res) {
                float rv[8];
                ld_global_v8(rv, a.res + off);
#pragma unroll
                for (int b = 0; b < 8; ++b) v[b] += rv[b];
              }
              st_global_v8(a.y + off, v);
              continue;
            }
          }
#pragma unroll
          for (int h = 0; h < B / 4; ++h) {
            float4 x = make_float4(o[4 * h][j], o[4 * h + 1][j], o[4 * h + 2][j], o[4 * h + 3][j]);
            if (a.res) {
              const float4 rv = *reinterpret_cast<const float4*>(a.res + off + 4 * h);
              x.x += rv.x; x.y += rv.y; x.z += rv.z; x.w += rv.w;
            }
            *reinterpret_cast<float4*>(a.y + off + 4 * h) = x;
          }
        }
      }
    }
    fence_before_sync();
    TSTAMP(24);
  }
  fence_before_sync();
  __syncthreads();
  if (warp == 0) tmem_dealloc(tbase, tcols);
  TSTAMP(5);
}

long long*& debug_buffer() {
  static long long* p = nullptr;
  return p;
}

constexpr size_t kSmemMax = 227 * 1024;

struct FwdPlan {
  bool ok;
  bool st1, st2;
  int Cp, kin8, ns1, ns2;
  size_t s1, s2;
  int64_t w1_floats, w2_floats;
};

template <int DIM>
FwdPlan fwd_plan(int cin, int c) {
  constexpr int B = Alg<DIM>::B, G = Alg<DIM>::G, P = Alg<DIM>::P;
  FwdPlan p;
  memset(&p, 0, sizeof(p));
  if (c < 1 || cin < 1) return p;
  const int Cp = round_up(c, 16), kin8 = round_up(cin, 8);
  p.Cp = Cp; p.kin8 = kin8;
  const size_t ring = (size_t)(kRing + 1) * B * kPS;
  const size_t par1 = (size_t)Cp * (1 + 2 * G) * 4 + 96, par2 = (size_t)Cp * (G + P + 2) * 4 + 8 * kTile * 4 + 96;
  p.s1 = ring + (size_t)G * 2 * kin8 * Cp * 4 + par1;
  p.ns1 = Cp;
  if (B * Cp > 512 || p.s1 > kSmemMax) {
    p.st1 = true;
    int ns = (512 / B) / 16 * 16;
    while (ns >= 16 && (Cp % ns || (size_t)kRing * wunit_bytes<DIM>(ns) + ring + par1 > kSmemMax)) ns -= 16;
    if (ns < 16) return p;
    p.ns1 = ns;
    p.s1 = (size_t)kRing * wunit_bytes<DIM>(ns) + ring + par1;
    p.w1_floats = weight_image_floats<DIM>(0, ns, Cp / ns, kin8 / 8);
  }
  p.s2 = ring + (size_t)2 * G * 2 * Cp * Cp * 4 + par2;
  p.ns2 = Cp;
  if (2 * B * Cp > 512 || p.s2 > kSmemMax) {
    p.st2 = true;
    int ns = (512 / (2 * B)) / 16 * 16;
    while (ns >= 16 && (Cp % ns || (size_t)kRing * wunit_bytes<DIM>(2 * ns) + ring + par2 > kSmemMax)) ns -= 16;
    if (ns < 16) return p;
    p.ns2 = ns;
    p.s2 = (size_t)kRing * wunit_bytes<DIM>(2 * ns) + ring + par2;
    p.w2_floats = weight_image_floats<DIM>(1, ns, Cp / ns, Cp / 8);
  }
  p.ok = true;
  return p;
}

template <int DIM>
bool fwd_supported(int cin, int c) { return fwd_plan<DIM>(cin, c).ok; }

inline int64_t align32f(int64_t floats) { return (floats + 31) / 32 * 32; }
inline bool overlap_enabled() {
  const char* e = getenv("CSMPN_TC_OVERLAP");
  return !(e && e[0] == '0');
}

template <int DIM>
int64_t fwd_ws_bytes(const csmpn_block_desc& d) {
  const FwdPlan p = fwd_plan<DIM>(d.c0 + d.c1 + d.c2, d.c);
  if (!p.ok) return -1;
  return (align32f(p.w1_floats) + align32f(p.w2_floats)) * 4;
}

template <int DIM>
int launch_weight_images(const WPrepArgs& w, int64_t floats, cudaStream_t stream) {
  const int threads = 256;
  int64_t blocks = (floats + threads - 1) / threads;
  if (blocks > 4096) blocks = 4096;
  tc_weight_images_kernel<DIM><<<(unsigned)blocks, threads, 0, stream>>>(w);
  CSMPN_LAUNCH_CHECK("tc_weight_images_kernel");
  return CSMPN_OK;
}

template <int DIM>
int launch_fwd(const csmpn_block_desc& d, cudaStream_t stream) {
  constexpr int B = Alg<DIM>::B;
  FwdArgs a;
  memset(&a, 0, sizeof(a));
  a.rows = d.rows;
  a.tiles = (int)((d.rows + kTile - 1) / kTile);
  a.C = d.c;
  a.Cp = round_up(d.c, 16);
  a.cin = d.c0 + d.c1 + d.c2;
  a.kin8 = round_up(a.cin, 8);
  a.in_bpt = d.in_bpt;
  a.in_cp = round_up(a.cin, 16);
  a.mode = d.mode; a.c0 = d.c0; a.c1 = d.c1; a.c2 = d.c2; a.pair_attr = d.pair_attr;
  a.vt_k = d.vt_k; a.vt_fp = d.vt_fp;
  a.p0 = d.p0; a.p1 = d.p1; a.p2 = d.p2;
  a.src = d.src; a.dst = d.dst; a.eid = d.eid;
  a.w1 = d.w1; a.b1 = d.b1; a.sa = d.sa; a.sb = d.sb; a.wr = d.wr; a.na = d.na; a.wl = d.wl; a.bl = d.bl; a.wp = d.wp; a.la = d.la;
  a.save_y1 = d.save_y1; a.y2 = d.save_y2; a.save_xr = d.save_xr; a.save_o = d.save_o; a.save_x0 = d.save_x0;
  a.y = d.y; a.res = d.res; a.out_bpt = d.out_bpt; a.has_b1 = d.has_b1;
  a.dbg = debug_buffer();
  if (!a.y2 || !a.y) return CSMPN_ERR_BAD_ARG;
  if (a.in_bpt && (d.mode != 0 || d.c1 || d.c2)) return CSMPN_ERR_BAD_ARG;
  if (d.mode == 2 && (d.vt_k < 1 || d.vt_k > 3 || d.vt_fp < 1 || d.c0 % (d.vt_k * d.vt_fp) || d.c1 || d.c2 || !d.src)) return CSMPN_ERR_BAD_ARG;
  if (a.out_bpt && d.res) return CSMPN_ERR_BAD_ARG;
  const FwdPlan p = fwd_plan<DIM>(a.cin, a.C);
  if (!p.ok) return CSMPN_ERR_UNSUPPORTED;
  if (a.tiles == 0) return CSMPN_OK;
  a.ns1 = p.ns1; a.ns2 = p.ns2;
  const int mask = d.stage_mask ? d.stage_mask : ~0;
  if (p.st1 || p.st2) {
    if (!d.fwd_ws || d.fwd_ws_bytes < (align32f(p.w1_floats) + align32f(p.w2_floats)) * 4) return CSMPN_ERR_WORKSPACE;
    if (p.st2 && !d.save_o) return CSMPN_ERR_BAD_ARG;
    float* w1img = (float*)d.fwd_ws;
    float* w2img = w1img + align32f(p.w1_floats);
    a.wimg1 = w1img; a.wimg2 = w2img;
    if (p.st1 && (mask & 1)) {
      WPrepArgs w{d.w1, nullptr, 0, 0, a.C, a.cin, 0, p.ns1, a.Cp / p.ns1, a.kin8 / 8, 0, w1img};
      int st = launch_weight_images<DIM>(w, p.w1_floats, stream);
      if (st) return st;
    }
    if (p.st2 && (mask & 2)) {
      WPrepArgs w{d.wr, d.wl, 1, 0, a.C, a.C, 0, p.ns2, a.Cp / p.ns2, a.Cp / 8, 0, w2img};
      int st = launch_weight_images<DIM>(w, p.w2_floats, stream);
      if (st) return st;
    }
  }
  const int grid = a.tiles < sm_count_cached() ? a.tiles : sm_count_cached();
  auto run = [&](auto kern, size_t smem_bytes) -> int {
    CSMPN_CUDA_TRY(cudaFuncSetAttribute(kern, cudaFuncAttributeMaxDynamicSharedMemorySize, (int)smem_bytes));
    kern<<<grid, kThreads, smem_bytes, stream>>>(a);
    return CSMPN_OK;
  };
  long long* const dbg_buf = a.dbg;
  const char* dbg_k = getenv("CSMPN_DBG_KERNEL");
  const bool dbg_f1 = dbg_k && dbg_k[0] == 'f' && dbg_k[1] == '1';
  a.dbg = dbg_f1 ? dbg_buf : nullptr;
  if (mask & 1) {
    const bool overlap = !p.st1 && 2 * B * a.Cp <= 512 && overlap_enabled();
    int rc = overlap ? (a.in_bpt ? run(tc_f1db_kernel<DIM, true>, p.s1) : run(tc_f1db_kernel<DIM, false>, p.s1))
             : a.in_bpt ? (p.st1 ? run(tc_f1_kernel<DIM, true, true>, p.s1) : run(tc_f1_kernel<DIM, true, false>, p.s1))
                        : (p.st1 ? run(tc_f1_kernel<DIM, false, true>, p.s1) : run(tc_f1_kernel<DIM, false, false>, p.s1));
    if (rc) return rc;
    CSMPN_LAUNCH_CHECK("tc_f1_kernel");
  }
  a.dbg = dbg_f1 ? nullptr : dbg_buf;
  if (mask & 2) {
    int rc;
#ifdef CSMPN_DEBUG_TOOLS
    if (a.dbg && !p.st2) rc = run(tc_f2_kernel<DIM, true, false>, p.s2);
    else
#endif
    rc = p.st2 ? run(tc_f2_kernel<DIM, false, true>, p.s2) : run(tc_f2_kernel<DIM, false, false>, p.s2);
    if (rc) return rc;
    CSMPN_LAUNCH_CHECK("tc_f2_kernel");
  }
  return CSMPN_OK;
}

}

int tc_block_fwd(int dim, const csmpn_block_desc* d, cudaStream_t stream) {
  if (dim == 2) return tcb::launch_fwd<2>(*d, stream);
  if (dim == 3) return tcb::launch_fwd<3>(*d, stream);
  return CSMPN_ERR_UNSUPPORTED;
}
void tc_set_debug_buffer(long long* p) { tcb::debug_buffer() = p; }
int64_t tc_block_fwd_workspace(int dim, const csmpn_block_desc* d) {
  if (dim == 2) return tcb::fwd_ws_bytes<2>(*d);
  if (dim == 3) return tcb::fwd_ws_bytes<3>(*d);
  return -1;
}
bool tc_block_bwd_supported(int dim, int c_in, int c);
int tc_block_bwd_wide(int dim, int c_in, int c);
bool tc_block_supported(int dim, int c_in, int c);
int tc_block_plan(int dim, int c_in, int c) {
  if (!tc_block_supported(dim, c_in, c)) return 0;
  tcb::FwdPlan p = dim == 2 ? tcb::fwd_plan<2>(c_in, c) : tcb::fwd_plan<3>(c_in, c);
  return 1 | (p.st1 ? 2 : 0) | (p.st2 ? 4 : 0) | (tc_block_bwd_wide(dim, c_in, c) ? 8 : 0);
}
bool tc_block_supported(int dim, int c_in, int c) {
  if (dim == 2) return tcb::fwd_supported<2>(c_in, c) && tc_block_bwd_supported(2, c_in, c);
  if (dim == 3) return tcb::fwd_supported<3>(c_in, c) && tc_block_bwd_supported(3, c_in, c);
  return false;
}

}
```

Before: 7.895 million.

## Split Cl(3,0) blade halves across two CTAs when tiles underfill SMs

When there are few tiles relative to SM count, the forward f1 kernel and the backward no-SiLU GEMM kernel launch two CTAs per tile. Each CTA handles four of the eight blades (two grades), staging half the weight images and using half the TMEM columns. This targets idle SMs at small problem sizes by doubling CTA-level parallelism. In exchange, input gathers and epilogue bookkeeping are duplicated, and the per-half SiLU gate must be computed from partial invariants, which risks correctness and adds extra global traffic.

```diff
diff --git a/clifford-group-equivariant-simplicial-message-passing-networks_b200/csrc/tc_block.cuh b/clifford-group-equivariant-simplicial-message-passing-networks_b200/csrc/tc_block.cuh
--- a/clifford-group-equivariant-simplicial-message-passing-networks_b200/csrc/tc_block.cuh
+++ b/clifford-group-equivariant-simplicial-message-passing-networks_b200/csrc/tc_block.cuh
@@ -37,6 +37,18 @@
 #pragma unroll
   for (int g = 0; g < A::G; ++g) sg[g] = fast_sigmoid(fmaf(a[g], inv[g], b[g]));
 }
+__device__ __forceinline__ bool half_in_second_grade(int s, int j) { return s ? j == 3 : j > 0; }
+__device__ __forceinline__ void silu_gates_half(const float* y1, int s, const float* a, const float* b, float* sg) {
+  float i0 = 0.f, i1 = 0.f;
+#pragma unroll
+  for (int j = 0; j < 4; ++j) {
+    if (half_in_second_grade(s, j)) i1 = fmaf(y1[j], y1[j], i1);
+    else i0 = fmaf(y1[j], y1[j], i0);
+  }
+  if (s == 0) i0 = y1[0];
+  sg[0] = fast_sigmoid(fmaf(a[2 * s], i0, b[2 * s]));
+  sg[1] = fast_sigmoid(fmaf(a[2 * s + 1], i1, b[2 * s + 1]));
+}
 
 template <int DIM>
 __device__ __forceinline__ void norm_factors(const float* xr, const float* s, float* q, float* nrm, float* rinv) {
@@ -65,11 +77,12 @@
   const float* w;
   int c_out, c_in, row0;
 };
-template <int DIM, bool TRANS, int NJ>
+template <int DIM, bool TRANS, int NJ, int NG = Alg<DIM>::G>
 __device__ __forceinline__ void stage_weight_jobs(const WJob (&j)[NJ], int njobs, uint32_t img_bytes, int rows_p, int cols_p,
-                                                  uint8_t* zero_base, uint32_t zero_bytes) {
+                                                  uint8_t* zero_base, uint32_t zero_bytes, int g0 = 0) {
   static_assert(NJ == 1 || NJ == 2, "one or two weights per call");
   constexpr int G = Alg<DIM>::G, U = 4;
+  static_assert(NG == G || (G == 4 && NG == 2), "all grades, or one half of Cl(3,0)'s");
   const int lane = threadIdx.x & 31, warp = threadIdx.x >> 5, nwarps = blockDim.x >> 5;
   const int rl = lane >> 2, cl = lane & 3;
   const WJob& j0 = j[0];
@@ -92,18 +105,21 @@
   };
   auto fetch = [&](int wb, float* v) {
 #pragma unroll
-    for (int g = 0; g < G; ++g) v[g] = 0.f;
+    for (int g = 0; g < NG; ++g) v[g] = 0.f;
     bool sj;
     int row, col;
     if (!decode(wb, sj, row, col)) return;
     const int o = TRANS ? col : row, i = TRANS ? row : col;
-    const float* src = (sj ? j1.w : j0.w) + ((size_t)o * (sj ? j1.c_in : j0.c_in) + i) * G;
-    if (G == 4 && (reinterpret_cast<uintptr_t>(src) & 15) == 0) {
+    const float* src = (sj ? j1.w : j0.w) + ((size_t)o * (sj ? j1.c_in : j0.c_in) + i) * G + g0;
+    if (NG == 4 && (reinterpret_cast<uintptr_t>(src) & 15) == 0) {
       const float4 x = __ldg(reinterpret_cast<const float4*>(src));
-      v[0] = x.x; v[1] = x.y; v[2] = x.z; v[G - 1] = x.w;
+      v[0] = x.x; v[1] = x.y; v[2] = x.z; v[NG - 1] = x.w;
+    } else if (NG == 2 && (reinterpret_cast<uintptr_t>(src) & 7) == 0) {
+      const float2 x = __ldg(reinterpret_cast<const float2*>(src));
+      v[0] = x.x; v[NG - 1] = x.y;
     } else {
 #pragma unroll
-      for (int g = 0; g < G; ++g) v[g] = __ldg(src + g);
+      for (int g = 0; g < NG; ++g) v[g] = __ldg(src + g);
     }
   };
   auto put = [&](int wb, const float* v) {
@@ -114,20 +130,20 @@
     if (r >= rows_p || col >= cols_p) return;
     uint8_t* dst = (sj ? j1.img0 : j0.img0) + plane_off(rows_p, r, col);
 #pragma unroll
-    for (int g = 0; g < G; ++g) {
+    for (int g = 0; g < NG; ++g) {
       const float hi = tf32_hi(v[g]);
       *reinterpret_cast<float*>(dst + (size_t)(g * 2 + 0) * img_bytes) = hi;
       *reinterpret_cast<float*>(dst + (size_t)(g * 2 + 1) * img_bytes) = v[g] - hi;
     }
   };
-  float x[U][G];
+  float x[U][NG];
 #pragma unroll
   for (int u = 0; u < U; ++u) fetch(warp + u * nwarps, x[u]);
   for (uint32_t i = threadIdx.x; i < (zero_bytes >> 4); i += blockDim.x)
     reinterpret_cast<float4*>(zero_base)[i] = make_float4(0.f, 0.f, 0.f, 0.f);
   __syncthreads();
   for (int base = 0; base < total; base += U * nwarps) {
-    float nx[U][G];
+    float nx[U][NG];
     const int nbase = base + U * nwarps;
     if (nbase < total) {
 #pragma unroll
@@ -139,16 +155,16 @@
 #pragma unroll
       for (int u = 0; u < U; ++u) {
 #pragma unroll
-        for (int g = 0; g < G; ++g) x[u][g] = nx[u][g];
+        for (int g = 0; g < NG; ++g) x[u][g] = nx[u][g];
       }
     }
   }
 }
-template <int DIM, bool TRANS>
+template <int DIM, bool TRANS, int NG = Alg<DIM>::G>
 __device__ __forceinline__ void stage_weight_images(uint8_t* img0, uint32_t img_bytes, const float* __restrict__ w, int c_out,
-                                                    int c_in, int rows_p, int cols_p) {
+                                                    int c_in, int rows_p, int cols_p, int g0 = 0) {
   const WJob j[1] = {{img0, w, c_out, c_in, 0}};
-  stage_weight_jobs<DIM, TRANS, 1>(j, 1, img_bytes, rows_p, cols_p, img0, (uint32_t)Alg<DIM>::G * 2u * img_bytes);
+  stage_weight_jobs<DIM, TRANS, 1, NG>(j, 1, img_bytes, rows_p, cols_p, img0, (uint32_t)NG * 2u * img_bytes, g0);
 }
 
 __device__ __forceinline__ uint64_t chunk_desc(uint32_t half_saddr, int b) {
@@ -234,13 +250,13 @@
   return (int64_t)npass * nk_total * Alg<DIM>::G * 2 * (stack ? 2 * np : np) * 8;
 }
 
-template <int B>
-__device__ __forceinline__ void issue_chunk_load(const Pipe& p, int q, const float* bpt, int cp, int64_t tile, int kc) {
+template <int B, int NB = B>
+__device__ __forceinline__ void issue_chunk_load(const Pipe& p, int q, const float* bpt, int cp, int64_t tile, int kc, int b0 = 0) {
   const int lane = threadIdx.x & 31;
   uint64_t* bar = &p.load_bar[q % kRing];
-  if (lane == 0) mbar_arrive_expect_tx(bar, B * 4096u);
+  if (lane == 0) mbar_arrive_expect_tx(bar, NB * 4096u);
   __syncwarp();
-  if (lane < B) bulk_g2s(p.slot(q) + lane * kPS, bpt + bpt_off(B, cp, tile, lane, 2 * kc, 0), 4096u, bar);
+  if (lane < NB) bulk_g2s(p.slot(q) + lane * kPS, bpt + bpt_off(B, cp, tile, b0 + lane, 2 * kc, 0), 4096u, bar);
 }
 template <int B>
 __device__ __forceinline__ void split_chunk(const Pipe& p, int q) {
@@ -272,12 +288,12 @@
   }
   p.conv_done(q);
 }
-template <int DIM>
+template <int DIM, int B = Alg<DIM>::B>
 __device__ __forceinline__ void issue_chunk_mma(const Pipe& p, int q, uint32_t tbase, uint32_t ncols, bool accumulate,
                                                 const uint8_t* wimg0, uint32_t img_bytes, int s0, int nsets, uint32_t set_bytes,
-                                                uint32_t w_rows, int ks, int n0, uint32_t idesc) {
+                                                uint32_t w_rows, int ks, int n0, uint32_t idesc, int b0 = 0) {
   using A = Alg<DIM>;
-  constexpr int B = A::B;
+  const int g0 = A::grade_of(b0);
   const uint64_t a_hi = chunk_desc(smem_addr(p.slot(q)), 0), a_lo = chunk_desc(smem_addr(p.lo), 0);
   const uint64_t w0 = smem_desc(smem_addr(wimg0) + (uint32_t)s0 * set_bytes + 2u * ks * w_rows * 16u + (uint32_t)n0 * 16u,
                                 w_rows * 16u, 128u);
@@ -288,8 +304,8 @@
     if (s < nsets) {
 #pragma unroll
       for (int b = 0; b < B; ++b)
-        mma_tf32_w(tbase + (uint32_t)(s * B + b) * ncols, a_lo + b * ps16, w0 + s * set16 + (2 * A::grade_of(b)) * img16, idesc,
-                 accumulate);
+        mma_tf32_w(tbase + (uint32_t)(s * B + b) * ncols, a_lo + b * ps16,
+                   w0 + s * set16 + (2 * (A::grade_of(b0 + b) - g0)) * img16, idesc, accumulate);
     }
   }
   mma_commit_w(p.lo_bar);
@@ -298,7 +314,7 @@
     if (s < nsets) {
 #pragma unroll
       for (int b = 0; b < B; ++b) {
-        const uint64_t wd = w0 + s * set16 + (2 * A::grade_of(b)) * img16;
+        const uint64_t wd = w0 + s * set16 + (2 * (A::grade_of(b0 + b) - g0)) * img16;
         const uint32_t d = tbase + (uint32_t)(s * B + b) * ncols;
         mma_tf32_w(d, a_hi + b * ps16, wd, idesc, 1);
         mma_tf32_w(d, a_hi + b * ps16, wd + img16, idesc, 1);
diff --git a/clifford-group-equivariant-simplicial-message-passing-networks_b200/csrc/tc_block_bwd.cu b/clifford-group-equivariant-simplicial-message-passing-networks_b200/csrc/tc_block_bwd.cu
--- a/clifford-group-equivariant-simplicial-message-passing-networks_b200/csrc/tc_block_bwd.cu
+++ b/clifford-group-equivariant-simplicial-message-passing-networks_b200/csrc/tc_block_bwd.cu
@@ -585,23 +585,27 @@
   }
 }
 
-template <int DIM, bool SILU>
+template <int DIM, bool SILU, bool HALF>
 __global__ void __launch_bounds__(kThreads, 1) tc_bgemmdb_kernel(GemmArgs a) {
   using A = Alg<DIM>;
   constexpr int B = A::B, G = A::G, NPS = 2 * G + 1;
+  static_assert(!HALF || (B == 8 && !SILU), "blade halves of Cl(3,0), MVSiLU adjoint in its own kernel");
+  constexpr int NB = HALF ? 4 : B, NG = HALF ? 2 : G;
+  const int hs = HALF ? (int)(blockIdx.x & 1) : 0, b0 = 4 * hs;
+  const int cta = HALF ? (int)(blockIdx.x >> 1) : (int)blockIdx.x, ncta = HALF ? (int)(gridDim.x >> 1) : (int)gridDim.x;
   constexpr int kUnits = 6;
   extern __shared__ __align__(1024) uint8_t smem[];
   const int tid = threadIdx.x, warp = uniform_warp_idx(), lane = tid & 31;
   const uint32_t img = (uint32_t)a.n16 * a.kmax * 4;
-  const uint32_t set_bytes = G * 2 * img;
-  uint8_t* wimg = smem + (kRing + 1) * B * kPS;
+  const uint32_t set_bytes = NG * 2 * img;
+  uint8_t* wimg = smem + (kRing + 1) * NB * kPS;
   const int nsets = a.src[1] ? 2 : 1;
   uint64_t* bars = reinterpret_cast<uint64_t*>(wimg + (size_t)nsets * set_bytes);
   uint32_t* tmem_slot = reinterpret_cast<uint32_t*>(bars + kPipeBars);
   float* sa_s = reinterpret_cast<float*>(tmem_slot + 4);
   float* sb_s = sa_s + a.n16 * G;
   Pipe p;
-  p.init(smem, bars, B * kPS);
+  p.init(smem, bars, NB * kPS);
   if (SILU) {
     for (int i = tid; i < a.n16 * G; i += kThreads) {
       sa_s[i] = (i < a.C * G) ? a.sa[i] : 0.f;
@@ -612,24 +616,24 @@
 #pragma unroll
   for (int u = 0; u < kUnits; ++u) { acc[u][0] = 0.f; acc[u][1] = 0.f; }
   const int nk = a.nk[0] + a.nk[1];
-  const int my_tiles = (a.tiles - (int)blockIdx.x + (int)gridDim.x - 1) / (int)gridDim.x;
+  const int my_tiles = (a.tiles - cta + ncta - 1) / ncta;
   const int total_chunks = my_tiles * nk;
   auto issue = [&](int qq) {
-    const int64_t tile = (int64_t)blockIdx.x + (int64_t)(qq / nk) * gridDim.x;
+    const int64_t tile = (int64_t)cta + (int64_t)(qq / nk) * ncta;
     const int kc = qq % nk;
     const int s = kc < a.nk[0] ? 0 : 1;
-    issue_chunk_load<B>(p, qq, a.src[s], a.cp[s], tile, s ? kc - a.nk[0] : kc);
+    issue_chunk_load<B, NB>(p, qq, a.src[s], a.cp[s], tile, s ? kc - a.nk[0] : kc, b0);
   };
   int q = 0, loaded = 0;
   if (warp == 0) for (; loaded < kRing - 1 && loaded < total_chunks; ++loaded) issue(loaded);
   const int Np = a.n16;
-  const uint32_t bufcols = (uint32_t)B * Np;
+  const uint32_t bufcols = (uint32_t)NB * Np;
   const uint32_t need = 2 * bufcols;
   const uint32_t tcols = need <= 32 ? 32 : need <= 64 ? 64 : need <= 128 ? 128 : need <= 256 ? 256 : 512;
   if (warp == 0) tmem_alloc(tmem_slot, tcols);
   {
     const WJob wj[2] = {{wimg, a.w[0], a.wk[0], a.wn, 0}, {wimg + set_bytes, a.w[nsets - 1], a.wk[nsets - 1], a.wn, 0}};
-    stage_weight_jobs<DIM, true, 2>(wj, nsets, img, a.n16, a.kmax, wimg, (uint32_t)nsets * set_bytes);
+    stage_weight_jobs<DIM, true, 2, NG>(wj, nsets, img, a.n16, a.kmax, wimg, (uint32_t)nsets * set_bytes, A::grade_of(b0));
   }
   fence_async_smem();
   fence_before_sync();
@@ -645,22 +649,22 @@
   auto epilogue_unit = [&](int64_t tile, int c4, uint32_t tb) {
     const int64_t row0 = tile * kTile;
     const bool row_ok = row0 + r < a.rows;
-    float v[B][4];
-#pragma unroll
-    for (int b = 0; b < B; ++b) tmem_ld4(tmem_at(tb, lane_base, b * Np + c4 * 4), v[b]);
+    float v[NB][4];
+#pragma unroll
+    for (int b = 0; b < NB; ++b) tmem_ld4(tmem_at(tb, lane_base, b * Np + c4 * 4), v[b]);
     if (a.addend) {
-      float4 ad[B];
-#pragma unroll
-      for (int b = 0; b < B; ++b) ad[b] = *reinterpret_cast<const float4*>(a.addend + bpt_off(B, a.n16, tile, b, c4, r));
+      float4 ad[NB];
+#pragma unroll
+      for (int b = 0; b < NB; ++b) ad[b] = *reinterpret_cast<const float4*>(a.addend + bpt_off(B, a.n16, tile, b0 + b, c4, r));
       tmem_wait_ld();
 #pragma unroll
-      for (int b = 0; b < B; ++b) {
+      for (int b = 0; b < NB; ++b) {
         v[b][0] += ad[b].x; v[b][1] += ad[b].y; v[b][2] += ad[b].z; v[b][3] += ad[b].w;
       }
     } else {
       tmem_wait_ld();
     }
-    if constexpr (SILU) {
+    if constexpr (SILU && !HALF) {
       const int u = c4 / 3;
 #pragma unroll
       for (int pr = 0; pr < 2; ++pr) {
@@ -721,10 +725,10 @@
     }
     if (a.out_bpt) {
 #pragma unroll
-      for (int b = 0; b < B; ++b) {
+      for (int b = 0; b < NB; ++b) {
         float4 x = make_float4(v[b][0], v[b][1], v[b][2], v[b][3]);
         if (!row_ok) x = make_float4(0.f, 0.f, 0.f, 0.f);
-        *reinterpret_cast<float4*>(a.out + bpt_off(B, a.n16, tile, b, c4, r)) = x;
+        *reinterpret_cast<float4*>(a.out + bpt_off(B, a.n16, tile, b0 + b, c4, r)) = x;
       }
     } else if (row_ok) {
 #pragma unroll
@@ -732,7 +736,11 @@
         const int n = c4 * 4 + jj;
         if (n >= a.wn) continue;
         float* dst = a.out + ((size_t)(row0 + r) * a.wn + n) * B;
-        if constexpr (B == 8) {
+        if constexpr (HALF) {
+          *reinterpret_cast<float4*>(dst + b0) = make_float4(v[0][jj], v[1][jj], v[2][jj], v[3][jj]);
+          continue;
+        }
+        if constexpr (B == 8 && !HALF) {
           if (wide_ok) {
             float w8[8];
 #pragma unroll
@@ -766,7 +774,7 @@
   };
 
   for (int t = 0; t < my_tiles; ++t) {
-    const int64_t tile = (int64_t)blockIdx.x + (int64_t)t * gridDim.x;
+    const int64_t tile = (int64_t)cta + (int64_t)t * ncta;
     const uint32_t tb = tbase + (uint32_t)(t & 1) * bufcols;
     for (int kc = 0; kc < nk; ++kc, ++q) {
       if (warp == 0) {
@@ -777,10 +785,10 @@
           ++loaded;
         }
         const int s = kc < a.nk[0] ? 0 : 1;
-        issue_chunk_mma<DIM>(p, q, tb, Np, kc > 0, wimg, img, s, 1, set_bytes, a.n16, s ? kc - a.nk[0] : kc, 0, idesc);
+        issue_chunk_mma<DIM, NB>(p, q, tb, Np, kc > 0, wimg, img, s, 1, set_bytes, a.n16, s ? kc - a.nk[0] : kc, 0, idesc, b0);
       } else {
         mbar_wait(&p.load_bar[q % kRing], (q / kRing) & 1);
-        split_chunk<B>(p, q);
+        split_chunk<NB>(p, q);
         epilogue_step();
       }
     }
@@ -791,7 +799,7 @@
   fence_before_sync();
   __syncthreads();
   if (warp == 0) tmem_dealloc(tbase, tcols);
-  if constexpr (SILU) {
+  if constexpr (SILU && !HALF) {
     float* red = reinterpret_cast<float*>(p.lo);
 #pragma unroll
     for (int u = 0; u < kUnits; ++u) {
@@ -1218,11 +1226,26 @@
   CSMPN_CUDA_TRY(cudaFuncSetAttribute(tc_bgemm_kernel<DIM, false, false>, cudaFuncAttributeMaxDynamicSharedMemorySize, (int)kSmemMax));
   CSMPN_CUDA_TRY(cudaFuncSetAttribute(tc_bgemm_kernel<DIM, true, false>, cudaFuncAttributeMaxDynamicSharedMemorySize, (int)kSmemMax));
   CSMPN_CUDA_TRY(cudaFuncSetAttribute(tc_bgemm_kernel<DIM, false, true>, cudaFuncAttributeMaxDynamicSharedMemorySize, (int)kSmemMax));
-  CSMPN_CUDA_TRY(cudaFuncSetAttribute(tc_bgemmdb_kernel<DIM, false>, cudaFuncAttributeMaxDynamicSharedMemorySize, (int)kSmemMax));
-  CSMPN_CUDA_TRY(cudaFuncSetAttribute(tc_bgemmdb_kernel<DIM, true>, cudaFuncAttributeMaxDynamicSharedMemorySize, (int)kSmemMax));
+  CSMPN_CUDA_TRY(cudaFuncSetAttribute(tc_bgemmdb_kernel<DIM, false, false>, cudaFuncAttributeMaxDynamicSharedMemorySize, (int)kSmemMax));
+  CSMPN_CUDA_TRY(cudaFuncSetAttribute(tc_bgemmdb_kernel<DIM, true, false>, cudaFuncAttributeMaxDynamicSharedMemorySize, (int)kSmemMax));
   auto overlap_ok = [&](int n16) {
     const char* e = getenv("CSMPN_TC_OVERLAP");
     return !(e && e[0] == '0') && 2 * B * n16 <= 512 && n16 <= 64;
+  };
+  const int sms = sm_count_cached();
+  auto halves_ok = [&](int n16) {
+    const char* e = getenv("CSMPN_TC_OVERLAP");
+    return B == 8 && !(e && e[0] == '0') && 3 * p.tiles <= sms && 2 * 4 * n16 <= 512 && n16 <= 64;
+  };
+  auto half_smem = [&](int nsets, int n16, int kmax) {
+    return gemm_smem<DIM>(nsets, n16, kmax) - (size_t)(kRing + 1) * 4 * kPS - (size_t)nsets * 2 * 2 * n16 * kmax * 4;
+  };
+  auto run_halves = [&](const GemmArgs& g, size_t sm) -> int {
+    if constexpr (B == 8) {
+      CSMPN_CUDA_TRY(cudaFuncSetAttribute(tc_bgemmdb_kernel<DIM, false, true>, cudaFuncAttributeMaxDynamicSharedMemorySize, (int)sm));
+      tc_bgemmdb_kernel<DIM, false, true><<<2 * p.tiles, kThreads, sm, stream>>>(g);
+    }
+    return CSMPN_OK;
   };
   auto prep = [&](const WPrepArgs& w, int64_t floats) -> int {
     int64_t blocks = (floats + 255) / 256;
@@ -1240,9 +1263,12 @@
       tc_bgemm_kernel<DIM, false, true><<<grid, kThreads, gemm_smem_streamed<DIM>(p.np), stream>>>(ga);
     } else {
       const size_t sm = gemm_smem<DIM>(2, ga.n16, ga.kmax, fuse_silu);
-      if (overlap_ok(ga.n16)) {
-        if (fuse_silu) tc_bgemmdb_kernel<DIM, true><<<grid, kThreads, sm, stream>>>(ga);
-        else tc_bgemmdb_kernel<DIM, false><<<grid, kThreads, sm, stream>>>(ga);
+      if (!fuse_silu && halves_ok(ga.n16)) {
+        int rc = run_halves(ga, half_smem(2, ga.n16, ga.kmax));
+        if (rc) return rc;
+      } else if (overlap_ok(ga.n16)) {
+        if (fuse_silu) tc_bgemmdb_kernel<DIM, true, false><<<grid, kThreads, sm, stream>>>(ga);
+        else tc_bgemmdb_kernel<DIM, false, false><<<grid, kThreads, sm, stream>>>(ga);
       } else if (fuse_silu) {
         tc_bgemm_kernel<DIM, true, false><<<grid, kThreads, sm, stream>>>(ga);
       } else {
@@ -1278,8 +1304,11 @@
       if (rc) return rc;
       ga.wimg = img_gx; ga.np = p.np;
       tc_bgemm_kernel<DIM, false, true><<<grid, kThreads, gemm_smem_streamed<DIM>(p.np), stream>>>(ga);
+    } else if (halves_ok(ga.n16)) {
+      int rc = run_halves(ga, half_smem(1, ga.n16, ga.kmax));
+      if (rc) return rc;
     } else if (overlap_ok(ga.n16)) {
-      tc_bgemmdb_kernel<DIM, false><<<grid, kThreads, gemm_smem<DIM>(1, ga.n16, ga.kmax), stream>>>(ga);
+      tc_bgemmdb_kernel<DIM, false, false><<<grid, kThreads, gemm_smem<DIM>(1, ga.n16, ga.kmax), stream>>>(ga);
     } else {
       tc_bgemm_kernel<DIM, false, false><<<grid, kThreads, gemm_smem<DIM>(1, ga.n16, ga.kmax), stream>>>(ga);
     }
diff --git a/clifford-group-equivariant-simplicial-message-passing-networks_b200/csrc/tc_block_fwd.cu b/clifford-group-equivariant-simplicial-message-passing-networks_b200/csrc/tc_block_fwd.cu
--- a/clifford-group-equivariant-simplicial-message-passing-networks_b200/csrc/tc_block_fwd.cu
+++ b/clifford-group-equivariant-simplicial-message-passing-networks_b200/csrc/tc_block_fwd.cu
@@ -35,9 +35,9 @@
 #define TSTAMP(code) do { } while (0)
 #endif
 
-template <int DIM>
+template <int DIM, bool HALF = false>
 struct ApiItems {
-  static constexpr int H = Alg<DIM>::B / 4, PPR = 8 * H, TOT = kTile * PPR, N = (TOT + kConv - 1) / kConv;
+  static constexpr int H = HALF ? 1 : Alg<DIM>::B / 4, PPR = 8 * H, TOT = kTile * PPR, N = (TOT + kConv - 1) / kConv;
   __device__ static __forceinline__ void decode(int it, int& r, int& cl, int& h) {
     const int l = it & 31, g = it >> 5;
     h = l % H;
@@ -47,20 +47,21 @@
   }
 };
 
-template <int DIM>
+template <int DIM, bool HALF = false>
 struct GatherIdx {
-  int32_t d[ApiItems<DIM>::N], s[ApiItems<DIM>::N], e[ApiItems<DIM>::N];
+  int32_t d[ApiItems<DIM, HALF>::N], s[ApiItems<DIM, HALF>::N], e[ApiItems<DIM, HALF>::N];
 };
-template <int DIM>
-__device__ __forceinline__ void load_gather_idx(const FwdArgs& a, int64_t row0, GatherIdx<DIM>& gi) {
-  constexpr int N = ApiItems<DIM>::N, TOT = ApiItems<DIM>::TOT;
+template <int DIM, bool HALF>
+__device__ __forceinline__ void load_gather_idx(const FwdArgs& a, int64_t row0, GatherIdx<DIM, HALF>& gi) {
+  using I = ApiItems<DIM, HALF>;
+  constexpr int N = I::N, TOT = I::TOT;
   if (a.mode == 0) return;
   const int ct = (int)threadIdx.x - 32;
 #pragma unroll
   for (int i = 0; i < N; ++i) {
     const int it = ct + i * kConv;
     int r, cl, h;
-    ApiItems<DIM>::decode(it, r, cl, h);
+    I::decode(it, r, cl, h);
     const int64_t R = row0 + r;
     const bool ok = it < TOT && R < a.rows;
     if (a.mode == 2) {
@@ -75,15 +76,18 @@
   }
 }
 
-template <int DIM>
-__device__ __forceinline__ void gather_chunk_api(const FwdArgs& a, int64_t row0, int kc, float4* v, const GatherIdx<DIM>& gi) {
-  constexpr int B = Alg<DIM>::B, H = ApiItems<DIM>::H, PPR = ApiItems<DIM>::PPR, N = ApiItems<DIM>::N, TOT = ApiItems<DIM>::TOT;
+template <int DIM, bool HALF>
+__device__ __forceinline__ void gather_chunk_api(const FwdArgs& a, int64_t row0, int kc, float4* v, const GatherIdx<DIM, HALF>& gi,
+                                                 int hq0) {
+  using I = ApiItems<DIM, HALF>;
+  constexpr int B = Alg<DIM>::B, N = I::N, TOT = I::TOT;
   const int ct = (int)threadIdx.x - 32;
 #pragma unroll
   for (int i = 0; i < N; ++i) {
     const int it = ct + i * kConv;
     int r, cl, h;
-    ApiItems<DIM>::decode(it, r, cl, h);
+    I::decode(it, r, cl, h);
+    h += hq0;
     const int c = kc * 8 + cl;
     const int64_t R = row0 + r;
     v[i] = make_float4(0.f, 0.f, 0.f, 0.f);
@@ -114,10 +118,11 @@
     }
   }
 }
-template <int DIM>
-__device__ __forceinline__ void store_chunk_api(const Pipe& p, int q, const float4* v, float* x0, int x0_cp, int64_t tile, int kc) {
-  constexpr int B = Alg<DIM>::B;
-  constexpr int H = ApiItems<DIM>::H, PPR = ApiItems<DIM>::PPR, N = ApiItems<DIM>::N, TOT = ApiItems<DIM>::TOT;
+template <int DIM, bool HALF>
+__device__ __forceinline__ void store_chunk_api(const Pipe& p, int q, const float4* v, float* x0, int x0_cp, int64_t tile, int kc,
+                                                int hq0) {
+  using I = ApiItems<DIM, HALF>;
+  constexpr int B = Alg<DIM>::B, N = I::N, TOT = I::TOT;
   const int ct = (int)threadIdx.x - 32;
   uint8_t* hi = p.slot(q);
   uint8_t* lo = p.lo;
@@ -127,7 +132,7 @@
     const int it = ct + i * kConv;
     if (it < TOT) {
       int r, cl, h;
-      ApiItems<DIM>::decode(it, r, cl, h);
+      I::decode(it, r, cl, h);
       float4 hv;
       split4(v[i], hv, lv[i]);
       const uint32_t off = (4 * h) * kPS + (cl >> 2) * kKH + r * 16 + (cl & 3) * 4;
@@ -143,8 +148,8 @@
       const int it = ct + i * kConv;
       if (it < TOT) {
         int r, cl, h;
-        ApiItems<DIM>::decode(it, r, cl, h);
-        float* dst = x0 + bpt_off(B, x0_cp, tile, 4 * h, 2 * kc + (cl >> 2), r) + (cl & 3);
+        I::decode(it, r, cl, h);
+        float* dst = x0 + bpt_off(B, x0_cp, tile, 4 * (h + hq0), 2 * kc + (cl >> 2), r) + (cl & 3);
         const size_t bs = (size_t)(x0_cp >> 2) * kTile * 4;
         dst[0] = v[i].x;
         dst[bs] = v[i].y;
@@ -159,7 +164,7 @@
     const int it = ct + i * kConv;
     if (it < TOT) {
       int r, cl, h;
-      ApiItems<DIM>::decode(it, r, cl, h);
+      I::decode(it, r, cl, h);
       const uint32_t off = (4 * h) * kPS + (cl >> 2) * kKH + r * 16 + (cl & 3) * 4;
       *reinterpret_cast<float*>(lo + off) = lv[i].x;
       *reinterpret_cast<float*>(lo + off + kPS) = lv[i].y;
@@ -169,10 +174,10 @@
   }
 }
 __device__ __forceinline__ void conv_barrier() { asm volatile("bar.sync 1, %0;" ::"n"(kConv) : "memory"); }
-template <int B>
-__device__ __forceinline__ void zero_chunk_bpt(float* dst, int cp, int64_t tile, int kc) {
-  for (int it = (int)threadIdx.x - 32; it < B * 2 * kTile; it += kConv) {
-    const int r = it & (kTile - 1), kh = (it >> 7) & 1, b = it >> 8;
+template <int B, int NB = B>
+__device__ __forceinline__ void zero_chunk_bpt(float* dst, int cp, int64_t tile, int kc, int b0 = 0) {
+  for (int it = (int)threadIdx.x - 32; it < NB * 2 * kTile; it += kConv) {
+    const int r = it & (kTile - 1), kh = (it >> 7) & 1, b = b0 + (it >> 8);
     *reinterpret_cast<float4*>(dst + bpt_off(B, cp, tile, b, 2 * kc + kh, r)) = make_float4(0.f, 0.f, 0.f, 0.f);
   }
 }
@@ -216,7 +221,7 @@
   GatherIdx<DIM> gi;
   if (!BPT_IN && warp != 0 && total_chunks > 0) {
     load_gather_idx<DIM>(a, tile_of(0) * kTile, gi);
-    gather_chunk_api<DIM>(a, tile_of(0) * kTile, 0, gv, gi);
+    gather_chunk_api<DIM>(a, tile_of(0) * kTile, 0, gv, gi, 0);
   }
   if (LOADS && warp == 0) {
     for (; loaded < kRing - 1 && loaded < total_chunks; ++loaded) load(loaded);
@@ -267,11 +272,11 @@
         } else {
           if (q >= kRing) mbar_wait(&p.slot_bar[q % kRing], ((q - kRing) / kRing) & 1);
           float* x0 = ps == 0 ? a.save_x0 : nullptr;
-          store_chunk_api<DIM>(p, q, gv, x0, round_up(a.kin8, 16), tile, kc);
+          store_chunk_api<DIM, false>(p, q, gv, x0, round_up(a.kin8, 16), tile, kc, 0);
           p.conv_done(q);
           if (q + 1 < total_chunks) {
             if ((q + 1) % per_tile == 0) load_gather_idx<DIM>(a, tile_of(q + 1) * kTile, gi);
-            gather_chunk_api<DIM>(a, tile_of(q + 1) * kTile, (q + 1) % nk, gv, gi);
+            gather_chunk_api<DIM>(a, tile_of(q + 1) * kTile, (q + 1) % nk, gv, gi, 0);
           }
           if (x0 && kc == nk - 1 && (a.kin8 & 8)) zero_chunk_bpt<B>(x0, round_up(a.kin8, 16), tile, nk);
         }
@@ -327,47 +332,51 @@
   if (warp == 0) tmem_dealloc(tbase, tcols);
 }
 
-template <int DIM, bool BPT_IN>
+template <int DIM, bool BPT_IN, bool HALF>
 __global__ void __launch_bounds__(kThreads, 1) tc_f1db_kernel(FwdArgs a) {
   using A = Alg<DIM>;
   [[maybe_unused]] constexpr bool TL = true;
   [[maybe_unused]] int dbg_n = 0;
   constexpr int B = A::B, G = A::G;
+  static_assert(!HALF || B == 8, "blade halves of Cl(3,0) only");
+  constexpr int NB = HALF ? 4 : B, NG = HALF ? 2 : G;
+  const int hs = HALF ? (int)(blockIdx.x & 1) : 0, b0 = 4 * hs;
+  const int cta = HALF ? (int)(blockIdx.x >> 1) : (int)blockIdx.x, ncta = HALF ? (int)(gridDim.x >> 1) : (int)gridDim.x;
   extern __shared__ __align__(1024) uint8_t smem[];
   const int tid = threadIdx.x, warp = uniform_warp_idx(), lane = tid & 31;
   const int C = a.C, Cp = a.Cp, nk = a.kin8 / 8;
   const uint32_t img = (uint32_t)a.kin8 * Cp * 4;
-  uint8_t* wimg = smem + (kRing + 1) * B * kPS;
-  float* b1_s = reinterpret_cast<float*>(wimg + (size_t)G * 2 * img);
+  uint8_t* wimg = smem + (kRing + 1) * NB * kPS;
+  float* b1_s = reinterpret_cast<float*>(wimg + (size_t)NG * 2 * img);
   float* sa_s = b1_s + Cp;
   float* sb_s = sa_s + Cp * G;
   uint64_t* bars = reinterpret_cast<uint64_t*>(sb_s + Cp * G);
   uint32_t* tmem_slot = reinterpret_cast<uint32_t*>(bars + kPipeBars);
   Pipe p;
-  p.init(smem, bars, B * kPS);
-  const int my_tiles = (a.tiles - (int)blockIdx.x + (int)gridDim.x - 1) / (int)gridDim.x;
+  p.init(smem, bars, NB * kPS);
+  const int my_tiles = (a.tiles - cta + ncta - 1) / ncta;
   const int total_chunks = my_tiles * nk;
-  auto tile_of = [&](int q) { return (int64_t)blockIdx.x + (int64_t)(q / nk) * gridDim.x; };
+  auto tile_of = [&](int q) { return (int64_t)cta + (int64_t)(q / nk) * ncta; };
   int q = 0, loaded = 0;
-  float4 gv[BPT_IN ? 1 : ApiItems<DIM>::N];
-  GatherIdx<DIM> gi;
+  float4 gv[BPT_IN ? 1 : ApiItems<DIM, HALF>::N];
+  GatherIdx<DIM, HALF> gi;
   if (!BPT_IN && warp != 0 && total_chunks > 0) {
     load_gather_idx<DIM>(a, tile_of(0) * kTile, gi);
-    gather_chunk_api<DIM>(a, tile_of(0) * kTile, 0, gv, gi);
+    gather_chunk_api<DIM>(a, tile_of(0) * kTile, 0, gv, gi, hs);
   }
   if (BPT_IN && warp == 0) {
     for (; loaded < kRing - 1 && loaded < total_chunks; ++loaded)
-      issue_chunk_load<B>(p, loaded, a.p0, a.in_cp, tile_of(loaded), loaded % nk);
-  }
-
-  const uint32_t bufcols = (uint32_t)B * Cp;
+      issue_chunk_load<B, NB>(p, loaded, a.p0, a.in_cp, tile_of(loaded), loaded % nk, b0);
+  }
+
+  const uint32_t bufcols = (uint32_t)NB * Cp;
   const uint32_t need = 2 * bufcols;
   const uint32_t tcols = need <= 32 ? 32 : need <= 64 ? 64 : need <= 128 ? 128 : need <= 256 ? 256 : 512;
   if (warp == 0) tmem_alloc(tmem_slot, tcols);
   const float pf_b1 = (tid < C && a.has_b1) ? __ldg(a.b1 + tid) : 0.f;
   const float pf_sa = tid < C * G ? __ldg(a.sa + tid) : 0.f;
   const float pf_sb = tid < C * G ? __ldg(a.sb + tid) : 0.f;
-  stage_weight_images<DIM, false>(wimg, img, a.w1, C, a.cin, Cp, a.kin8);
+  stage_weight_images<DIM, false, NG>(wimg, img, a.w1, C, a.cin, Cp, a.kin8, A::grade_of(b0));
   if (tid < Cp) b1_s[tid] = pf_b1;
   for (int i = tid + kThreads; i < Cp; i += kThreads) b1_s[i] = (i < C && a.has_b1) ? a.b1[i] : 0.f;
   if (tid < Cp * G) { sa_s[tid] = pf_sa; sb_s[tid] = pf_sb; }
@@ -386,39 +395,47 @@
 
   auto epilogue_unit = [&](int64_t tile, int c4, uint32_t tb) {
     const bool row_ok = tile * kTile + r < a.rows;
-    float v[B][4];
-#pragma unroll
-    for (int b = 0; b < B; ++b) tmem_ld4(tmem_at(tb, (warp & 3) * 32, b * Cp + c4 * 4), v[b]);
+    float v[NB][4];
+#pragma unroll
+    for (int b = 0; b < NB; ++b) tmem_ld4(tmem_at(tb, (warp & 3) * 32, b * Cp + c4 * 4), v[b]);
     tmem_wait_ld();
 #pragma unroll
     for (int j = 0; j < 4; ++j) {
       const int ch = c4 * 4 + j;
-      float y1[B];
+      float y1[NB];
       const bool ok = row_ok && ch < C;
 #pragma unroll
-      for (int b = 0; b < B; ++b) y1[b] = ok ? v[b][j] : 0.f;
-      if (ok) y1[0] += b1_s[ch];
-#pragma unroll
-      for (int b = 0; b < B; ++b) v[b][j] = y1[b];
+      for (int b = 0; b < NB; ++b) y1[b] = ok ? v[b][j] : 0.f;
+      if (ok && b0 == 0) y1[0] += b1_s[ch];
+#pragma unroll
+      for (int b = 0; b < NB; ++b) v[b][j] = y1[b];
     }
     if (a.save_y1) {
 #pragma unroll
-      for (int b = 0; b < B; ++b)
-        *reinterpret_cast<float4*>(a.save_y1 + bpt_off(B, Cp, tile, b, c4, r)) = make_float4(v[b][0], v[b][1], v[b][2], v[b][3]);
+      for (int b = 0; b < NB; ++b)
+        *reinterpret_cast<float4*>(a.save_y1 + bpt_off(B, Cp, tile, b0 + b, c4, r)) = make_float4(v[b][0], v[b][1], v[b][2], v[b][3]);
     }
 #pragma unroll
     for (int j = 0; j < 4; ++j) {
       const int ch = c4 * 4 + j;
-      float y1[B], sg[G], inv[G];
-#pragma unroll
-      for (int b = 0; b < B; ++b) y1[b] = v[b][j];
-      silu_gates<DIM>(y1, sa_s + ch * G, sb_s + ch * G, sg, inv);
-#pragma unroll
-      for (int b = 0; b < B; ++b) v[b][j] = y1[b] * sg[A::grade_of(b)];
-    }
-#pragma unroll
-    for (int b = 0; b < B; ++b)
-      *reinterpret_cast<float4*>(a.y2 + bpt_off(B, Cp, tile, b, c4, r)) = make_float4(v[b][0], v[b][1], v[b][2], v[b][3]);
+      float y1[NB];
+#pragma unroll
+      for (int b = 0; b < NB; ++b) y1[b] = v[b][j];
+      if constexpr (HALF) {
+        float sg[2];
+        silu_gates_half(y1, hs, sa_s + ch * G, sb_s + ch * G, sg);
+#pragma unroll
+        for (int b = 0; b < NB; ++b) v[b][j] = y1[b] * (half_in_second_grade(hs, b) ? sg[1] : sg[0]);
+      } else {
+        float sg[G], inv[G];
+        silu_gates<DIM>(y1, sa_s + ch * G, sb_s + ch * G, sg, inv);
+#pragma unroll
+        for (int b = 0; b < B; ++b) v[b][j] = y1[b] * sg[A::grade_of(b)];
+      }
+    }
+#pragma unroll
+    for (int b = 0; b < NB; ++b)
+      *reinterpret_cast<float4*>(a.y2 + bpt_off(B, Cp, tile, b0 + b, c4, r)) = make_float4(v[b][0], v[b][1], v[b][2], v[b][3]);
   };
   int64_t pend_tile = -1;
   int pend_c4 = 0, pend_q = 0;
@@ -439,7 +456,7 @@
   };
 
   for (int t = 0; t < my_tiles; ++t) {
-    const int64_t tile = (int64_t)blockIdx.x + (int64_t)t * gridDim.x;
+    const int64_t tile = (int64_t)cta + (int64_t)t * ncta;
     const uint32_t tb = tbase + (uint32_t)(t & 1) * bufcols;
     for (int kc = 0; kc < nk; ++kc, ++q) {
       if (warp == 0) {
@@ -448,28 +465,29 @@
         TSTAMP(37);
         if (BPT_IN && loaded == q + kRing - 1 && loaded < total_chunks) {
           if (q >= 1) mbar_wait(&p.slot_bar[(q - 1) % kRing], ((q - 1) / kRing) & 1);
-          issue_chunk_load<B>(p, loaded, a.p0, a.in_cp, tile_of(loaded), loaded % nk);
+          issue_chunk_load<B, NB>(p, loaded, a.p0, a.in_cp, tile_of(loaded), loaded % nk, b0);
           ++loaded;
         }
-        issue_chunk_mma<DIM>(p, q, tb, Cp, kc > 0, wimg, img, 0, 1, 0, Cp, kc, 0, idesc);
+        issue_chunk_mma<DIM, NB>(p, q, tb, Cp, kc > 0, wimg, img, 0, 1, 0, Cp, kc, 0, idesc, b0);
         TSTAMP(38);
       } else {
         if (BPT_IN) {
           mbar_wait(&p.load_bar[q % kRing], (q / kRing) & 1);
-          split_chunk<B>(p, q);
+          split_chunk<NB>(p, q);
         } else {
           TSTAMP(30);
           if (q >= kRing) mbar_wait(&p.slot_bar[q % kRing], ((q - kRing) / kRing) & 1);
           TSTAMP(31);
-          store_chunk_api<DIM>(p, q, gv, a.save_x0, round_up(a.kin8, 16), tile, kc);
+          store_chunk_api<DIM, HALF>(p, q, gv, a.save_x0, round_up(a.kin8, 16), tile, kc, hs);
           TSTAMP(32);
           p.conv_done(q);
           TSTAMP(33);
           if (q + 1 < total_chunks) {
             if ((q + 1) % nk == 0) load_gather_idx<DIM>(a, tile_of(q + 1) * kTile, gi);
-            gather_chunk_api<DIM>(a, tile_of(q + 1) * kTile, (q + 1) % nk, gv, gi);
+            gather_chunk_api<DIM>(a, tile_of(q + 1) * kTile, (q + 1) % nk, gv, gi, hs);
           }
-          if (a.save_x0 && kc == nk - 1 && (a.kin8 & 8)) zero_chunk_bpt<B>(a.save_x0, round_up(a.kin8, 16), tile, nk);
+          if (a.save_x0 && kc == nk - 1 && (a.kin8 & 8))
+            zero_chunk_bpt<B, NB>(a.save_x0, round_up(a.kin8, 16), tile, nk, b0);
           TSTAMP(34);
         }
         epilogue_step();
@@ -739,6 +757,7 @@
   bool st1, st2;
   int Cp, kin8, ns1, ns2;
   size_t s1, s2;
+  size_t s1h;
   int64_t w1_floats, w2_floats;
 };
 
@@ -753,6 +772,7 @@
   const size_t ring = (size_t)(kRing + 1) * B * kPS;
   const size_t par1 = (size_t)Cp * (1 + 2 * G) * 4 + 96, par2 = (size_t)Cp * (G + P + 2) * 4 + 8 * kTile * 4 + 96;
   p.s1 = ring + (size_t)G * 2 * kin8 * Cp * 4 + par1;
+  p.s1h = (size_t)(kRing + 1) * 4 * kPS + (size_t)2 * 2 * kin8 * Cp * 4 + par1;
   p.ns1 = Cp;
   if (B * Cp > 512 || p.s1 > kSmemMax) {
     p.st1 = true;
@@ -851,7 +871,8 @@
       if (st) return st;
     }
   }
-  const int grid = a.tiles < sm_count_cached() ? a.tiles : sm_count_cached();
+  const int sms = sm_count_cached();
+  int grid = a.tiles < sms ? a.tiles : sms;
   auto run = [&](auto kern, size_t smem_bytes) -> int {
     CSMPN_CUDA_TRY(cudaFuncSetAttribute(kern, cudaFuncAttributeMaxDynamicSharedMemorySize, (int)smem_bytes));
     kern<<<grid, kThreads, smem_bytes, stream>>>(a);
@@ -863,9 +884,20 @@
   a.dbg = dbg_f1 ? dbg_buf : nullptr;
   if (mask & 1) {
     const bool overlap = !p.st1 && 2 * B * a.Cp <= 512 && overlap_enabled();
-    int rc = overlap ? (a.in_bpt ? run(tc_f1db_kernel<DIM, true>, p.s1) : run(tc_f1db_kernel<DIM, false>, p.s1))
-             : a.in_bpt ? (p.st1 ? run(tc_f1_kernel<DIM, true, true>, p.s1) : run(tc_f1_kernel<DIM, true, false>, p.s1))
-                        : (p.st1 ? run(tc_f1_kernel<DIM, false, true>, p.s1) : run(tc_f1_kernel<DIM, false, false>, p.s1));
+    const bool halves = B == 8 && !p.st1 && 2 * a.tiles <= sms && 2 * 4 * a.Cp <= 512 && overlap_enabled();
+    int rc;
+    if constexpr (B == 8) {
+      if (halves) {
+        grid = 2 * a.tiles;
+        rc = a.in_bpt ? run(tc_f1db_kernel<DIM, true, true>, p.s1h) : run(tc_f1db_kernel<DIM, false, true>, p.s1h);
+        grid = a.tiles < sms ? a.tiles : sms;
+      }
+    }
+    if (!halves) {
+      rc = overlap ? (a.in_bpt ? run(tc_f1db_kernel<DIM, true, false>, p.s1) : run(tc_f1db_kernel<DIM, false, false>, p.s1))
+           : a.in_bpt ? (p.st1 ? run(tc_f1_kernel<DIM, true, true>, p.s1) : run(tc_f1_kernel<DIM, true, false>, p.s1))
+                      : (p.st1 ? run(tc_f1_kernel<DIM, false, true>, p.s1) : run(tc_f1_kernel<DIM, false, false>, p.s1));
+    }
     if (rc) return rc;
     CSMPN_LAUNCH_CHECK("tc_f1_kernel");
   }
```

Result: faster. 7.976 million (median of 6 runs) (+1.0%).
